# eglrp/PSBA

Measured on AMD Instinct MI355X. Metric: M-observations/sec through Jacobian+Schur build+solve (ms/LM-iter in ms_per_step), higher is better.
Workload: dtype f64; 1 GPU; venice-shaped; n_cams=52, n_pts=64053, n_obs=345364, lm=levmar, TR hand-off disabled, parallelism=points sharded x1

## Files before the change

### include/psba_hip.h

```cpp
#ifndef PSBA_HIP_H
#define PSBA_HIP_H

#ifdef __cplusplus
extern "C" {
#endif

typedef struct psba_ctx *psba_handle;

#define PSBA_OK 0
#define PSBA_NOT_SPD 1
#define PSBA_SINGULAR_V 2
#define PSBA_PCG_MAXIT 4
#define PSBA_E_INVALID (-1)
#define PSBA_E_HIP (-2)
#define PSBA_E_RCCL (-3)
#define PSBA_E_IO (-4)
#define PSBA_E_NOMEM (-5)
#define PSBA_E_STATE (-6)

#define PSBA_ITER_TURN_TO_LM 1
#define PSBA_ITER_TURN_TO_TR 2
#define PSBA_ITER_CONTINUE 3
#define PSBA_ITER_ERR 4
#define PSBA_ITER_DP_NO_CHANGE 5
// ... 117 lines not shown
int psba_set_step(psba_handle h, const double *dp);
int psba_cholmod_lambda(psba_handle h, int reassemble, double *lambda, double *info3);
int psba_get_cholmod_factor(psba_handle h, double *L);
int psba_get_free_obs_blocks(psba_handle h, double *W, double *Be);

typedef struct {
  int max_iter;
  int start_itno;
  int verbose;
  int log_cap;
  double init_lambda;
} psba_tr_options;

typedef struct {
  int flag;
  int iters;
  int tries;
  int chol_fail;
  double init_err, final_err, lambda, delta;
  int n_log;
  double seconds;
} psba_tr_result;

void psba_tr_default_options(psba_tr_options *o);
int psba_trust_region(psba_handle h, const psba_tr_options *opts, psba_tr_result *res, double *log);

typedef struct {
  int flag, iters, lm_calls, tr_calls;
  double init_err, final_err, seconds;
} psba_solve_result;
int psba_solve(psba_handle h, int max_iter, int verbose, psba_solve_result *res);

int psba_partition_points(int n3Dpts, const int *iidx, int n2Dprojs, int nranks, int *pt_begin);
int psba_comm_unique_id(void *id128);
int psba_comm_init(psba_handle h, int nranks, int rank, const void *id128);
int psba_comm_rank(psba_handle h, int *nranks, int *rank);
int psba_set_rank_layout(psba_handle h, int nranks, int rank);
int psba_reduce_buffer_size(psba_handle h, long long *n_doubles);
int psba_get_reduce_buffer(psba_handle h, double *out);
int psba_set_reduce_buffer(psba_handle h, const double *in);

typedef struct {
  int nCams, n3Dpts, n2Dprojs;
  double *Kparas, *impts, *initrot, *camsEx, *pts3D;
  int *iidx, *jidx;
} psba_problem;
int psba_read_problem(const char *cams_file, const char *pts_file, const double *fixedK,
                      psba_problem *out);
void psba_free_problem(psba_problem *p);
typedef struct {
  psba_problem base;
  double *kc, *cov;
} psba_problem_ex;
int psba_read_problem_ex(const char *cams_file, const char *pts_file, const double *fixedK, psba_problem_ex *out);
void psba_free_problem_ex(psba_problem_ex *p);
int psba_write_problem(const char *cams_file, const char *pts_file, int nCams, int n3Dpts, int n2Dprojs,
                       const double *Kparas, const double *initrot, const double *camsEx, const double *pts3D,
                       const double *impts, const int *iidx, const int *jidx, int with_K);
int psba_convert_bal(const char *bal_file, const char *cams_out, const char *pts_out, double *max_abs_k);
int psba_convert_bal_kd(const char *bal_file, const char *cams_out, const char *pts_out);

#define PSBA_K_LINEARIZE 0
#define PSBA_K_SCHUR 1
#define PSBA_K_CHOLESKY 2
#define PSBA_K_BACKSUB 3
#define PSBA_K_RESIDUAL 4
#define PSBA_K_ALLREDUCE 5
#define PSBA_K_SCHUR_REDUCE 6
#define PSBA_K_COUNT 7
int psba_profile_enable(psba_handle h, int on);
int psba_profile_reset(psba_handle h);
int psba_profile_get(psba_handle h, int kernel, double *total_ms, int *launches);
int psba_algorithmic_bytes(psba_handle h, int kernel, double *bytes);

#define PSBA_SOLVER_DENSE 0
#define PSBA_SOLVER_PCG 1
int psba_set_solver(psba_handle h, int solver, double tol, int max_iter);
int psba_pcg_info(psba_handle h, int *iters, double *relres, long long *blocks, long long *dense_blocks);
int psba_get_sparse_S(psba_handle h, int *jk, double *val, double *ea);
int psba_set_sparse_S(psba_handle h, const double *val, const double *ea);
int psba_sparse_pattern(int nCams, int n3Dpts, int n2Dprojs, const int *iidx, const int *jidx, unsigned char *flags);
int psba_set_sparse_pattern(psba_handle h, const unsigned char *flags, long long n);

int psba_chol_dist_shape(psba_handle h, int *n32, int *NB, int *sharded);
int psba_chol_shape(psba_handle h, int *out8);
int psba_chol_dist_exchange_plan(int n32, int NB, int nranks, int JE, long long *out4, int cap);
int psba_chol_dist_begin(psba_handle h);
int psba_chol_dist_superpanel(psba_handle h, int J);
int psba_chol_dist_block(psba_handle h, int B, int set, double *buf, long long *n_doubles);
int psba_chol_dist_finish(psba_handle h);

typedef struct psba_schur_plan *psba_schur_plan_t;
psba_schur_plan_t psba_schur_plan_create(int nCams, int n3Dpts, int n2Dprojs, const int *iidx,
                                         const int *jidx);
int psba_schur_plan_info(psba_schur_plan_t p, long long info[8]);
int psba_schur_plan_copy(psba_schur_plan_t p, unsigned long long *items, long long *wg,
                         int *blockpos, int *glo);
void psba_schur_plan_destroy(psba_schur_plan_t p);

typedef struct psba_owner_plan *psba_owner_plan_t;
psba_owner_plan_t psba_owner_plan_create(int nCams, int n3Dpts, int n2Dprojs, const int *iidx, const int *jidx,
                                         const unsigned char *pattern);
int psba_owner_plan_info(psba_owner_plan_t p, long long info[4]);
int psba_owner_plan_copy(psba_owner_plan_t p, long long *waves, int *units, int *prod, int *blocks, int *diag_slot);
void psba_owner_plan_destroy(psba_owner_plan_t p);

typedef struct psba_blockprod_plan *psba_blockprod_plan_t;
psba_blockprod_plan_t psba_blockprod_plan_create(int nCams, int n3Dpts, int n2Dprojs, const int *iidx, const int *jidx,
                                                 int seg_len);
int psba_blockprod_plan_info(psba_blockprod_plan_t p, long long info[4]);
int psba_blockprod_plan_copy(psba_blockprod_plan_t p, int *blocks, int *segs, int *prods);
void psba_blockprod_plan_destroy(psba_blockprod_plan_t p);

#ifdef PSBA_BUILD_EXPERIMENTS
typedef struct psba_ring_plan *psba_ring_plan_t;
psba_ring_plan_t psba_ring_plan_create(int nCams, int n3Dpts, int n2Dprojs, const int *iidx,
                                       const int *jidx);
int psba_ring_plan_info(psba_ring_plan_t p, long long info[16]);
int psba_ring_plan_copy(psba_ring_plan_t p, long long *wg, int *steps, unsigned *entries, int *ops,
                        int *jobs, int *lane_blk, int *blk_lane0, int *rb);
void psba_ring_plan_destroy(psba_ring_plan_t p);
#endif

#ifdef __cplusplus
}
#endif
#endif
```

### psba_amd/capi.py

```python
import ctypes as C
import os

import numpy as np

_HERE = os.path.dirname(os.path.abspath(__file__))
lib_path = os.environ.get("PSBA_LIB") or os.path.join(_HERE, "libpsba_hip.so")

if not os.path.exists(lib_path):
    raise ImportError(
        f"{lib_path} is missing: build the HIP extension first (python -m psba_amd.build, or "
        "__graft_entry__.build()). psba_amd has no CPU fallback.")
lib = C.CDLL(lib_path)

PSBA_OK, PSBA_NOT_SPD, PSBA_SINGULAR_V = 0, 1, 2
PARAMS_CUR, PARAMS_NEW = 0, 1
LOSS_NONE, LOSS_HUBER, LOSS_CAUCHY, LOSS_SOFT_L1 = 0, 1, 2, 3
CAMERA_FIXED_K, CAMERA_FREE_K, CAMERA_FREE_KD = 0, 1, 2
INTRINSICS_BAL = (1, 0, 0, 0, 0, 1, 1, 0, 0, 0)
ITER_TURN_TO_LM, ITER_TURN_TO_TR, ITER_CONTINUE, ITER_ERR = 1, 2, 3, 4
ITER_DP_NO_CHANGE, ITER_ERR_SMALL_ENOUGH, ITER_PASS = 5, 6, 7
K_LINEARIZE, K_SCHUR, K_CHOLESKY, K_BACKSUB, K_RESIDUAL, K_ALLREDUCE, K_SCHUR_REDUCE = range(7)
KERNEL_NAMES = ["linearize", "schur", "cholesky", "backsub", "residual", "allreduce", "schur_reduce"]

_h = C.c_void_p
# ... 41 lines not shown


class CProblemEx(C.Structure):
    _fields_ = [("base", CProblem), ("kc", _dp), ("cov", _dp)]


SIGNATURES = [
    ("psba_create", C.c_int, [C.c_int, C.POINTER(_h)]),
    ("psba_destroy", C.c_int, [_h]),
    ("psba_last_error", C.c_char_p, [_h]),
    ("psba_version", C.c_char_p, []),
    ("psba_upload_problem", C.c_int, [_h, C.c_int, C.c_int, C.c_int, _dp, _dp, _dp, _dp, _dp, _ip, _ip]),
    ("psba_set_params", C.c_int, [_h, _dp, _dp]),
    ("psba_reset_params", C.c_int, [_h]),
    ("psba_get_params", C.c_int, [_h, C.c_int, _dp, _dp]),
    ("psba_get_dims", C.c_int, [_h, _ip, _ip, _ip]),
    ("psba_schur_path", C.c_int, [_h, C.POINTER(C.c_int)]),
    ("psba_residual", C.c_int, [_h, C.c_int, _dp]),
    ("psba_linearize", C.c_int, [_h, C.c_double, C.c_double]),
    ("psba_max_diag", C.c_int, [_h, _dp]),
    ("psba_begin", C.c_int, [_h, C.c_double, C.c_double, _dp, _dp]),
    ("psba_schur_assemble", C.c_int, [_h, C.c_double]),
    ("psba_schur_reduce", C.c_int, [_h]),
    ("psba_schur_solve", C.c_int, [_h]),
    ("psba_backsub", C.c_int, [_h, C.c_double, C.POINTER(TryScalars)]),
    ("psba_backsub_async", C.c_int, [_h, C.c_double]),
    ("psba_linearize_ahead", C.c_int, [_h]),
    ("psba_backsub_wait", C.c_int, [_h, C.POINTER(TryScalars)]),
    ("psba_accept", C.c_int, [_h]),
    ("psba_compute_exQT", C.c_int, [_h, C.c_int, _dp]),
    ("psba_compute_jacobiQT", C.c_int, [_h, _dp, _dp]),
    ("psba_compute_U", C.c_int, [_h, C.c_double, _dp]),
    ("psba_compute_V", C.c_int, [_h, C.c_double, _dp]),
    ("psba_maxElmOfUV", C.c_int, [_h, _dp]),
    ("psba_update_UV", C.c_int, [_h, C.c_double, _dp, _dp]),
    ("psba_restore_UVdiag", C.c_int, [_h]),
    ("psba_compute_Vinv", C.c_int, [_h, _dp]),
    ("psba_compute_Wblks", C.c_int, [_h, C.c_double, _dp]),
    ("psba_compute_Yblks", C.c_int, [_h, _dp]),
    ("psba_compute_S", C.c_int, [_h, _dp]),
    ("psba_compute_g", C.c_int, [_h, C.c_double, _dp]),
    ("psba_compute_ea", C.c_int, [_h, _dp]),
    ("psba_SPDinv_matVec", C.c_int, [_h, _dp]),
    ("psba_compute_eb", C.c_int, [_h, _dp]),
    ("psba_compute_dpb", C.c_int, [_h, _dp]),
    ("psba_compute_newp", C.c_int, [_h, _dp]),
    ("psba_update_p", C.c_int, [_h, _dp]),
    ("psba_lm_default_options", None, [C.POINTER(LmOptions)]),
    ("psba_levmar", C.c_int, [_h, C.POINTER(LmOptions), C.POINTER(LmResult), _dp]),
    ("psba_partition_points", C.c_int, [C.c_int, _ip, C.c_int, C.c_int, _ip]),
    ("psba_comm_unique_id", C.c_int, [C.c_void_p]),
    ("psba_comm_init", C.c_int, [_h, C.c_int, C.c_int, C.c_void_p]),
    ("psba_comm_rank", C.c_int, [_h, _ip, _ip]),
    ("psba_set_rank_layout", C.c_int, [_h, C.c_int, C.c_int]),
    ("psba_reduce_buffer_size", C.c_int, [_h, C.POINTER(C.c_longlong)]),
    ("psba_get_reduce_buffer", C.c_int, [_h, _dp]),
    ("psba_set_reduce_buffer", C.c_int, [_h, _dp]),
    ("psba_read_problem", C.c_int, [C.c_char_p, C.c_char_p, _dp, C.POINTER(CProblem)]),
    ("psba_free_problem", None, [C.POINTER(CProblem)]),
    ("psba_profile_enable", C.c_int, [_h, C.c_int]),
    ("psba_profile_reset", C.c_int, [_h]),
    ("psba_profile_get", C.c_int, [_h, C.c_int, _dp, _ip]),
    ("psba_algorithmic_bytes", C.c_int, [_h, C.c_int, _dp]),
    ("psba_compute_Jmultiply", C.c_int, [_h, _dp, _dp]),
    ("psba_jmul_dots", C.c_int, [_h, _dp, _dp, _dp]),
    ("psba_get_gradient", C.c_int, [_h, _dp]),
    ("psba_get_dp", C.c_int, [_h, _dp]),
    ("psba_set_step", C.c_int, [_h, _dp]),
    ("psba_cholmod_lambda", C.c_int, [_h, C.c_int, _dp, _dp]),
    ("psba_get_cholmod_factor", C.c_int, [_h, _dp]),
    ("psba_get_free_obs_blocks", C.c_int, [_h, _dp, _dp]),
    ("psba_tr_default_options", None, [C.POINTER(TrOptions)]),
    ("psba_trust_region", C.c_int, [_h, C.POINTER(TrOptions), C.POINTER(TrResult), _dp]),
    ("psba_solve", C.c_int, [_h, C.c_int, C.c_int, C.POINTER(SolveResult)]),
    ("psba_write_problem", C.c_int, [C.c_char_p, C.c_char_p, C.c_int, C.c_int, C.c_int, _dp, _dp, _dp, _dp, _dp, _ip, _ip, C.c_int]),
    ("psba_convert_bal", C.c_int, [C.c_char_p, C.c_char_p, C.c_char_p, _dp]),
    ("psba_allreduce_scalars", C.c_int, [_h, _dp, C.c_int]),
    ("psba_set_solver", C.c_int, [_h, C.c_int, C.c_double, C.c_int]),
    ("psba_pcg_info", C.c_int, [_h, _ip, _dp, C.POINTER(C.c_longlong), C.POINTER(C.c_longlong)]),
    ("psba_get_sparse_S", C.c_int, [_h, _ip, _dp, _dp]),
    ("psba_set_sparse_S", C.c_int, [_h, _dp, _dp]),
    ("psba_sparse_pattern", C.c_int, [C.c_int, C.c_int, C.c_int, _ip, _ip, C.POINTER(C.c_ubyte)]),
    ("psba_set_sparse_pattern", C.c_int, [_h, C.POINTER(C.c_ubyte), C.c_longlong]),
    ("psba_set_camera_model", C.c_int, [_h, C.c_int]),
    ("psba_camera_block", C.c_int, [_h, _ip]),
    ("psba_set_distortion", C.c_int, [_h, _dp]),
    ("psba_set_obs_covariance", C.c_int, [_h, _dp]),
    ("psba_lens_model", C.c_int, [_h, _ip, _ip]),
    ("psba_set_robust_loss", C.c_int, [_h, C.c_int, C.c_double]),
    ("psba_robust_loss", C.c_int, [_h, _ip, _dp]),
    ("psba_obs_sq_residuals", C.c_int, [_h, C.c_int, _dp]),
    ("psba_set_fixed", C.c_int, [_h, C.POINTER(C.c_ubyte), C.POINTER(C.c_ubyte)]),
    ("psba_fixed_counts", C.c_int, [_h, _ip, _ip]),
    ("psba_read_problem_ex", C.c_int, [C.c_char_p, C.c_char_p, _dp, C.POINTER(CProblemEx)]),
    ("psba_free_problem_ex", None, [C.POINTER(CProblemEx)]),
    ("psba_convert_bal_kd", C.c_int, [C.c_char_p, C.c_char_p, C.c_char_p]),
    ("psba_chol_dist_exchange_plan", C.c_int, [C.c_int, C.c_int, C.c_int, C.c_int, C.POINTER(C.c_longlong), C.c_int]),
    ("psba_chol_dist_shape", C.c_int, [_h, _ip, _ip, _ip]),
    ("psba_chol_shape", C.c_int, [_h, _ip]),
    ("psba_chol_dist_begin", C.c_int, [_h]),
    ("psba_chol_dist_superpanel", C.c_int, [_h, C.c_int]),
    ("psba_chol_dist_block", C.c_int, [_h, C.c_int, C.c_int, _dp, C.POINTER(C.c_longlong)]),
    ("psba_chol_dist_finish", C.c_int, [_h]),
    ("psba_schur_plan_create", C.c_void_p, [C.c_int, C.c_int, C.c_int, _ip, _ip]),
    ("psba_schur_plan_info", C.c_int, [C.c_void_p, C.POINTER(C.c_longlong)]),
    ("psba_schur_plan_copy", C.c_int, [C.c_void_p, C.POINTER(C.c_ulonglong), C.POINTER(C.c_longlong), _ip, _ip]),
    ("psba_schur_plan_destroy", None, [C.c_void_p]),
    ("psba_owner_plan_create", C.c_void_p, [C.c_int, C.c_int, C.c_int, _ip, _ip, C.POINTER(C.c_ubyte)]),
    ("psba_owner_plan_info", C.c_int, [C.c_void_p, C.POINTER(C.c_longlong)]),
    ("psba_owner_plan_copy", C.c_int, [C.c_void_p, C.POINTER(C.c_longlong), _ip, _ip, _ip, _ip]),
    ("psba_owner_plan_destroy", None, [C.c_void_p]),
    ("psba_set_intrinsics_mask", C.c_int, [_h, C.POINTER(C.c_ubyte)]),
    ("psba_intrinsics_mask", C.c_int, [_h, C.POINTER(C.c_ubyte)]),
    ("psba_set_intrinsics_groups", C.c_int, [_h, C.POINTER(C.c_int)]),
    ("psba_intrinsics_groups", C.c_int, [_h, C.POINTER(C.c_int), C.POINTER(C.c_int)]),
    ("psba_blockprod_plan_create", C.c_void_p, [C.c_int, C.c_int, C.c_int, _ip, _ip, C.c_int]),
    ("psba_blockprod_plan_info", C.c_int, [C.c_void_p, C.POINTER(C.c_longlong)]),
    ("psba_blockprod_plan_copy", C.c_int, [C.c_void_p, _ip, _ip, _ip]),
    ("psba_blockprod_plan_destroy", None, [C.c_void_p]),
]
EXPERIMENT_SIGNATURES = [
    ("psba_ring_plan_create", C.c_void_p, [C.c_int, C.c_int, C.c_int, _ip, _ip]),
    ("psba_ring_plan_info", C.c_int, [C.c_void_p, C.POINTER(C.c_longlong)]),
    ("psba_ring_plan_copy", C.c_int, [C.c_void_p, C.POINTER(C.c_longlong), _ip, C.POINTER(C.c_uint), _ip, _ip, _ip, _ip, _ip]),
    ("psba_ring_plan_destroy", None, [C.c_void_p]),
]
HAS_EXPERIMENTS = hasattr(lib, "psba_ring_plan_create")
for _name, _res, _args in SIGNATURES + (EXPERIMENT_SIGNATURES if HAS_EXPERIMENTS else []):
    _f = getattr(lib, _name)
    _f.restype = _res
    _f.argtypes = _args


class PsbaError(RuntimeError):
    def __init__(self, code, msg):
        super().__init__(f"psba error {code}: {msg}")
        self.code = code


def _d(a):
    return None if a is None else a.ctypes.data_as(_dp)


def _i(a):
    return None if a is None else a.ctypes.data_as(_ip)


def _c(a, dt=np.float64):
    return np.ascontiguousarray(a, dtype=dt)


class Problem(dict):
    """K[nC,5] initrot[nC,4] cams[nC,6] pts[nP,3] impts[nO,2] iidx[nO] jidx[nO] nC nP nO.
    Optional: kc[nC,5], cov[nO,2,2] (read_problem_ex); fixed_cams[nC], fixed_pts[nP] (masks for Psba.set_fixed)."""


def sparse_pattern(prob):
    nC = int(prob["nC"])
    flags = np.zeros(nC * (nC + 1) // 2, dtype=np.uint8)
    ii = np.ascontiguousarray(prob["iidx"], dtype=np.int32)
    jj = np.ascontiguousarray(prob["jidx"], dtype=np.int32)
    rc = lib.psba_sparse_pattern(nC, int(prob["nP"]), int(prob["nO"]), _i(ii), _i(jj),
                                 flags.ctypes.data_as(C.POINTER(C.c_ubyte)))
    if rc != 0:
        raise PsbaError(rc, "psba_sparse_pattern failed")
    return flags


def _problem_from(cp):
    nC, nP, nO = cp.nCams, cp.n3Dpts, cp.n2Dprojs
    arr = lambda p, n, shape: np.ctypeslib.as_array(p, shape=(n,)).copy().reshape(shape)
    return Problem(K=arr(cp.Kparas, 5 * nC, (nC, 5)), initrot=arr(cp.initrot, 4 * nC, (nC, 4)),
                  cams=arr(cp.camsEx, 6 * nC, (nC, 6)), pts=arr(cp.pts3D, 3 * nP, (nP, 3)),
                  impts=arr(cp.impts, 2 * nO, (nO, 2)), iidx=arr(cp.iidx, nO, (nO,)).astype(np.int32),
                  jidx=arr(cp.jidx, nO, (nO,)).astype(np.int32), nC=nC, nP=nP, nO=nO)


def read_problem(cams_file, pts_file, fixedK=None):
    cp = CProblem()
    k = None if fixedK is None else _c(fixedK)
    rc = lib.psba_read_problem(os.fsencode(cams_file), os.fsencode(pts_file), _d(k), C.byref(cp))
    if rc != 0:
        raise PsbaError(rc, f"psba_read_problem({cams_file}, {pts_file}) failed")
    out = _problem_from(cp)
    lib.psba_free_problem(C.byref(cp))
    return out


def read_problem_ex(cams_file, pts_file, fixedK=None):
    cp = CProblemEx()
    k = None if fixedK is None else _c(fixedK)
    rc = lib.psba_read_problem_ex(os.fsencode(cams_file), os.fsencode(pts_file), _d(k), C.byref(cp))
    if rc != 0:
        raise PsbaError(rc, f"psba_read_problem_ex({cams_file}, {pts_file}) failed")
    out = _problem_from(cp.base)
    nC, nO = out["nC"], out["nO"]
    out["kc"] = np.ctypeslib.as_array(cp.kc, shape=(5 * nC,)).copy().reshape(nC, 5) if cp.kc else None
    out["cov"] = np.ctypeslib.as_array(cp.cov, shape=(4 * nO,)).copy().reshape(nO, 2, 2) if cp.cov else None
    lib.psba_free_problem_ex(C.byref(cp))
    return out


def write_problem(cams_file, pts_file, prob, cams=None, pts=None, with_K=True):
    c = _c(prob["cams"] if cams is None else cams)
    p = _c(prob["pts"] if pts is None else pts)
    K, rot, im = _c(prob["K"]), _c(prob["initrot"]), _c(prob["impts"])
    ii, jj = _c(prob["iidx"], np.int32), _c(prob["jidx"], np.int32)
    rc = lib.psba_write_problem(cams_file.encode(), pts_file.encode(), int(prob["nC"]), int(prob["nP"]),
                                int(prob["nO"]), _d(K), _d(rot), _d(c), _d(p), _d(im), _i(ii), _i(jj), int(with_K))
    if rc != 0:
        raise PsbaError(rc, f"psba_write_problem({cams_file}, {pts_file}) failed")


def convert_bal(bal_file, cams_out, pts_out):
    k = C.c_double()
    rc = lib.psba_convert_bal(bal_file.encode(), cams_out.encode(), pts_out.encode(), C.byref(k))
    if rc != 0:
        raise PsbaError(rc, f"psba_convert_bal({bal_file}) failed")
    return k.value


def convert_bal_kd(bal_file, cams_out, pts_out):
    rc = lib.psba_convert_bal_kd(bal_file.encode(), cams_out.encode(), pts_out.encode())
    if rc != 0:
        raise PsbaError(rc, f"psba_convert_bal_kd({bal_file}) failed")


def partition_points(n_pts, iidx, nranks):
    iidx = _c(iidx, np.int32)
    out = np.zeros(nranks + 1, dtype=np.int32)
    rc = lib.psba_partition_points(int(n_pts), _i(iidx), int(iidx.size), int(nranks), _i(out))
    if rc != 0:
        raise PsbaError(rc, "psba_partition_points failed")
    return out


def schur_plan(n_cams, n_pts, iidx, jidx):
    iidx = _c(iidx, np.int32)
    jidx = _c(jidx, np.int32)
    p = lib.psba_schur_plan_create(int(n_cams), int(n_pts), int(iidx.size), _i(iidx), _i(jidx))
    if not p:
        raise PsbaError(-1, "psba_schur_plan_create failed")
    try:
        info = (C.c_longlong * 8)()
        lib.psba_schur_plan_info(p, info)
        groups, nwg, nslots, products, slab, nblocks, run_tasks, pair_items = (int(x) for x in info)
        items = np.zeros(nslots, dtype=np.uint64)
        wg = np.zeros((nwg, 8), dtype=np.int64)
        blockpos = np.zeros(nblocks, dtype=np.int32)
        glo = np.zeros(groups + 1, dtype=np.int32)
        lib.psba_schur_plan_copy(p, items.ctypes.data_as(C.POINTER(C.c_ulonglong)),
                                 wg.ctypes.data_as(C.POINTER(C.c_longlong)), _i(blockpos), _i(glo))
    finally:
        lib.psba_schur_plan_destroy(p)
    return dict(groups=groups, items=items, wg=wg, blockpos=blockpos, glo=glo, products=products,
                slab_doubles=slab, run_tasks=run_tasks, pair_items=pair_items)


def owner_plan(n_cams, n_pts, iidx, jidx, pattern=None):
    iidx = _c(iidx, np.int32)
    jidx = _c(jidx, np.int32)
    pat = None if pattern is None else np.ascontiguousarray(pattern, dtype=np.uint8)
    pp = None if pat is None else pat.ctypes.data_as(C.POINTER(C.c_ubyte))
    p = lib.psba_owner_plan_create(int(n_cams), int(n_pts), int(iidx.size), _i(iidx), _i(jidx), pp)
    if not p:
        raise PsbaError(-1, "psba_owner_plan_create failed")
    try:
        info = (C.c_longlong * 4)()
        lib.psba_owner_plan_info(p, info)
        nw, rows, products, nblk = (int(x) for x in info)
        waves = np.zeros((nw, 2), dtype=np.int64)
        units = np.zeros((64 * nw, 4), dtype=np.int32)
        prod = np.zeros((64 * rows, 2), dtype=np.int32)
        blocks = np.zeros((nblk, 2), dtype=np.int32)
        diag = np.zeros(int(n_cams), dtype=np.int32)
        lib.psba_owner_plan_copy(p, waves.ctypes.data_as(C.POINTER(C.c_longlong)), _i(units), _i(prod), _i(blocks), _i(diag))
    finally:
        lib.psba_owner_plan_destroy(p)
    return dict(waves=waves, units=units, prod=prod.reshape(rows, 64, 2), blocks=blocks, diag_slot=diag, products=products)


def blockprod_plan(n_cams, n_pts, iidx, jidx, seg_len):
    iidx = _c(iidx, np.int32)
    jidx = _c(jidx, np.int32)
    p = lib.psba_blockprod_plan_create(int(n_cams), int(n_pts), int(iidx.size), _i(iidx), _i(jidx), int(seg_len))
    if not p:
        raise PsbaError(-1, "psba_blockprod_plan_create failed")
    try:
        info = (C.c_longlong * 4)()
        lib.psba_blockprod_plan_info(p, info)
        nb, ns, npr, tiles = (int(x) for x in info)
        blocks = np.zeros((nb, 2), dtype=np.int32)
        segs = np.zeros((ns, 3), dtype=np.int32)
        prods = np.zeros((npr, 2), dtype=np.int32)
        lib.psba_blockprod_plan_copy(p, _i(blocks), _i(segs), _i(prods))
    finally:
        lib.psba_blockprod_plan_destroy(p)
    return dict(blocks=blocks, segs=segs, prods=prods, tiles=tiles)


def chol_dist_exchange_plan(n32, NB, nranks, JE):
    out = np.zeros((64, 4), dtype=np.int64)
    n = lib.psba_chol_dist_exchange_plan(int(n32), int(NB), int(nranks), int(JE), out.ctypes.data_as(C.POINTER(C.c_longlong)), 64)
    if n < 0:
        raise PsbaError(n, "psba_chol_dist_exchange_plan failed")
    return [tuple(int(v) for v in row) for row in out[:n]]


def ring_plan(n_cams, n_pts, iidx, jidx):
    if not HAS_EXPERIMENTS:
# ... 146 lines not shown
        return c.value, p.value

    def obs_sq_residuals(self, which=PARAMS_CUR):
        return self._out(lib.psba_obs_sq_residuals, self.nO, which)[1]

    def camera_block(self):
        n = C.c_int()
        self._ck(lib.psba_camera_block(self._h, C.byref(n)))
        return n.value

    def upload_problem(self, prob):
        self.nC, self.nP, self.nO = int(prob["nC"]), int(prob["nP"]), int(prob["nO"])
        self.cnp = self.camera_block()
        self.nA, self.nB = self.cnp * self.nC, 3 * self.nP
        self.nT = self.nA + self.nB
        a = [_c(prob[k]).reshape(-1) for k in ("K", "impts", "initrot", "cams", "pts")]
        ii, jj = _c(prob["iidx"], np.int32), _c(prob["jidx"], np.int32)
        self._ck(lib.psba_upload_problem(self._h, self.nC, self.nP, self.nO, _d(a[0]), _d(a[1]),
                                         _d(a[2]), _d(a[3]), _d(a[4]), _i(ii), _i(jj)))

    def set_params(self, cams, pts):
        c, p = _c(cams).reshape(-1), _c(pts).reshape(-1)
        self._ck(lib.psba_set_params(self._h, _d(c), _d(p)))

    def reset_params(self):
        self._ck(lib.psba_reset_params(self._h))

    def get_params(self, which=PARAMS_CUR):
        c, p = np.empty(self.nA), np.empty(self.nB)
        self._ck(lib.psba_get_params(self._h, which, _d(c), _d(p)))
        return c.reshape(self.nC, self.cnp), p.reshape(self.nP, 3)

    def schur_path(self):
        v = C.c_int()
        self._ck(lib.psba_schur_path(self._h, C.byref(v)))
        return v.value

    def residual(self, which=PARAMS_CUR):
        v = C.c_double()
        self._ck(lib.psba_residual(self._h, which, C.byref(v)))
        return v.value

    def linearize(self, coeff=1.0, coeff_g=1.0):
        self._ck(lib.psba_linearize(self._h, coeff, coeff_g))

    def begin(self, coeff=1.0, coeff_g=1.0):
        c, m = C.c_double(), C.c_double()
        self._ck(lib.psba_begin(self._h, coeff, coeff_g, C.byref(c), C.byref(m)))
        return c.value, m.value

    def max_diag(self):
        v = C.c_double()
        self._ck(lib.psba_max_diag(self._h, C.byref(v)))
        return v.value

    def schur_assemble(self, mu):
        self._ck(lib.psba_schur_assemble(self._h, mu))

    def schur_reduce(self):
        self._ck(lib.psba_schur_reduce(self._h))

    def schur_solve(self):
        return self._ck(lib.psba_schur_solve(self._h))

    def backsub(self, mu):
        s = TryScalars()
        self._ck(lib.psba_backsub(self._h, mu, C.byref(s)))
        return s

    def backsub_async(self, mu):
        self._ck(lib.psba_backsub_async(self._h, mu))

    def linearize_ahead(self):
        self._ck(lib.psba_linearize_ahead(self._h))

    def backsub_wait(self):
        s = TryScalars()
        self._ck(lib.psba_backsub_wait(self._h, C.byref(s)))
        return s

    def accept(self):
        self._ck(lib.psba_accept(self._h))

    def _out(self, fn, n, *pre):
        out = np.empty(n)
        rc = self._ck(fn(self._h, *pre, _d(out)))
        return rc, out

    def compute_exQT(self, which=PARAMS_CUR):
        return self._out(lib.psba_compute_exQT, 2 * self.nO, which)[1]

    def compute_jacobiQT(self):
        JA, JB = np.empty(12 * self.nO), np.empty(6 * self.nO)
        self._ck(lib.psba_compute_jacobiQT(self._h, _d(JA), _d(JB)))
        return JA, JB

    def compute_U(self, coeff=1.0):
        return self._out(lib.psba_compute_U, 36 * self.nC, coeff)[1]

    def compute_V(self, coeff=1.0):
        return self._out(lib.psba_compute_V, 9 * self.nP, coeff)[1]

    def maxElmOfUV(self):
        v = C.c_double()
        self._ck(lib.psba_maxElmOfUV(self._h, C.byref(v)))
        return v.value

    def update_UV(self, mu):
        U, V = np.empty(36 * self.nC), np.empty(9 * self.nP)
        self._ck(lib.psba_update_UV(self._h, mu, _d(U), _d(V)))
        return U, V

    def restore_UVdiag(self):
        self._ck(lib.psba_restore_UVdiag(self._h))

    def compute_Vinv(self):
        return self._out(lib.psba_compute_Vinv, 9 * self.nP)

    def compute_Wblks(self, coeff=1.0):
        return self._out(lib.psba_compute_Wblks, 18 * self.nO, coeff)[1]

    def compute_Yblks(self):
        return self._out(lib.psba_compute_Yblks, 18 * self.nO)[1]

    def compute_S(self):
        return self._out(lib.psba_compute_S, self.nA * self.nA)[1].reshape(self.nA, self.nA)

    def compute_g(self, coeff=1.0):
        return self._out(lib.psba_compute_g, self.nT, coeff)[1]

    def compute_ea(self):
        return self._out(lib.psba_compute_ea, self.nA)[1]

    def SPDinv_matVec(self):
        return self._out(lib.psba_SPDinv_matVec, self.nA)

    def compute_eb(self):
        return self._out(lib.psba_compute_eb, self.nB)[1]

    def compute_dpb(self):
        return self._out(lib.psba_compute_dpb, self.nT)[1]

    def compute_newp(self):
        return self._out(lib.psba_compute_newp, self.nT)[1]

    def update_p(self):
        return self._out(lib.psba_update_p, self.nT)[1]

    def levmar(self, max_iter=50, tr_handoff=False, verbose=False, log_cap=512, start_itno=0, init_mu=0.0,
               stop_cost=0.0):
        opts = LmOptions(max_iter, int(tr_handoff), int(verbose), log_cap, start_itno, init_mu, stop_cost)
        res = LmResult()
        log = np.zeros((max(log_cap, 1), 5))
        self._ck(lib.psba_levmar(self._h, C.byref(opts), C.byref(res), _d(log)))
        return res, log[: res.n_log].copy()

    def set_solver(self, solver, tol=0.0, max_iter=0):
        self._ck(lib.psba_set_solver(self._h, int(solver), float(tol), int(max_iter)))

    def pcg_info(self):
        it, rr, nb, nd = C.c_int(), C.c_double(), C.c_longlong(), C.c_longlong()
        self._ck(lib.psba_pcg_info(self._h, C.byref(it), C.byref(rr), C.byref(nb), C.byref(nd)))
        return it.value, rr.value, nb.value, nd.value

    def get_sparse_S(self):
        nb = self.pcg_info()[2]
# ... 137 lines not shown
```

### psba_amd/csrc/kernels_backsub.hip

```cpp
#include <cstdlib>

#include "camera_model.h"
#include "psba_internal.h"

namespace psba {

struct BackArgs {
  const double *W, *PV, *camconst, *cams, *pts, *impts, *ga;
  const int *iidx, *jidx, *ptr;
  const int4 *tile_desc;
  double *dp;
  double *newcams, *newpts;
  double *scal;
  double *dbg_eb;
  const int *status;
  double mu;
  double coeff;
  int nC, nA, nTiles;
  int cam_terms;
  int mode;
  const double *kc, *wl;
};

template <bool DUMP, bool RECOMP, int LM>
// ... 249 lines not shown
    lens_load_w<LM>(p.wl, a, wl);
    const double2 m = reinterpret_cast<const double2 *>(p.impts)[a];
    lens_residual<LM>(cc, cam, sNP, kc, wl, m.x, m.y, e0, e1);
    s_cost += lens_cost<LM>(rl, e0, e1);
  }
  __syncthreads();
  {
    double v = s_cost;
#pragma unroll
    for (int off = 32; off > 0; off >>= 1) v += __shfl_down(v, off, 64);
    if ((tid & 63) == 0) sRed[tid >> 6][3] = v;
  }
  __syncthreads();
  if (tid == 0) {
    double c = 0.0;
    for (int w2 = 0; w2 < TILE_OBS / 64; w2++) c += sRed[w2][3];
    double *dst = p.scal + SC_PART + 4 * (blockIdx.x % SC_NPART);
    atomicAdd(&dst[0], s_dp);
    atomicAdd(&dst[1], s_den);
    atomicAdd(&dst[2], c);
    atomicAdd(&dst[3], s_np);
  }
}

__global__ __launch_bounds__(128) void k_publish_scal(const double *scal, double *host) {
  if (threadIdx.x < NSCAL) host[threadIdx.x] = scal[threadIdx.x];
}

int launch_publish_scal(psba_ctx *h, hipStream_t s) {
  hipLaunchKernelGGL(k_publish_scal, dim3(1), dim3(128), 0, s, h->scal, h->h_scal_dev);
  PSBA_HIP(h, hipGetLastError());
  return PSBA_OK;
}

__global__ __launch_bounds__(256) void k_struct_only_begin(const double *PV, double mu, int nA, int nP, double *dp, double *scal,
                                                           int *status, int try_id) {
  const int gtid = blockIdx.x * blockDim.x + threadIdx.x, gsize = gridDim.x * blockDim.x;
  if (blockIdx.x == 0 && threadIdx.x < 4 * SC_NPART) scal[SC_PART + threadIdx.x] = 0.0;
  if (blockIdx.x == 0 && threadIdx.x == 64) status[3] = try_id;
  for (int t = gtid; t < nA; t += gsize) dp[t] = 0.0;
  for (int i = gtid; i < nP; i += gsize) {
    double v[6], vi[6];
#pragma unroll
    for (int k = 0; k < 6; k++) v[k] = PV[9 * (size_t)i + k];
    v[0] += mu;
    v[3] += mu;
    v[5] += mu;
    if (sym3_inverse(v, vi)) status[0] = try_id;
  }
}

int launch_struct_only_try(psba_ctx *h, double mu) {
  h->try_id++;
  h->diag_done = false;
  h->packed_pending = false;
  int grid = (h->d.nP + 255) / 256;
  if (grid > 1024) grid = 1024;
  hipLaunchKernelGGL(k_struct_only_begin, dim3(grid), dim3(256), 0, h->stream, h->PV, mu, h->d.nA, h->d.nP, h->dp, h->scal,
                     h->status, h->try_id);
  PSBA_HIP(h, hipGetLastError());
  return PSBA_OK;
}

template <int LM>
static void enqueue_backsub(psba_ctx *h, const BackArgs &a, const RobustLoss &rl, const FixedMask &fm, int grid, bool dump, bool read_w) {
  if (dump && read_w)
    hipLaunchKernelGGL((k_backsub<true, false, LM>), dim3(grid), dim3(TILE_OBS), 0, h->stream, a, rl, fm);
  else if (dump)
    hipLaunchKernelGGL((k_backsub<true, true, LM>), dim3(grid), dim3(TILE_OBS), 0, h->stream, a, rl, fm);
  else if (read_w)
    hipLaunchKernelGGL((k_backsub<false, false, LM>), dim3(grid), dim3(TILE_OBS), 0, h->stream, a, rl, fm);
  else
    hipLaunchKernelGGL((k_backsub<false, true, LM>), dim3(grid), dim3(TILE_OBS), 0, h->stream, a, rl, fm);
  if (h->nLong) {
    if (dump)
      hipLaunchKernelGGL((k_backsub_long<true, LM>), dim3(h->nLong), dim3(TILE_OBS), 0, h->stream, a, h->long_pts, rl, fm);
    else
      hipLaunchKernelGGL((k_backsub_long<false, LM>), dim3(h->nLong), dim3(TILE_OBS), 0, h->stream, a, h->long_pts, rl, fm);
  }
}

int launch_backsub(psba_ctx *h, double mu, bool dump) {
  if (h->cnp != 6) return dump ? mirror_refused(h) : launch_backsub_free(h, mu);
  const Dims &d = h->d;
  BackArgs a;
  a.W = h->W;
  a.PV = h->PV;
  a.camconst = h->camconst;
  a.cams = h->cams[h->cur];
  a.pts = h->pts[h->cur];
  a.impts = h->impts;
  a.ga = h->ga;
  a.iidx = h->iidx;
  a.jidx = h->jidx;
  a.ptr = h->ptr;
  a.tile_desc = h->tile_desc;
  a.dp = h->dp;
  a.newcams = h->cams[1 - h->cur];
  a.newpts = h->pts[1 - h->cur];
  a.scal = h->scal;
  a.dbg_eb = h->dbg_eb;
  a.status = h->status;
  a.mu = mu;
  a.coeff = h->coeff_w;
  a.nC = d.nC;
  a.nA = d.nA;
  a.nTiles = d.nTiles;
  a.cam_terms = h->rank == 0 ? 1 : 0;
  a.kc = h->lens_kc;
  a.wl = h->lens_w;
  const RobustLoss rl = make_robust_loss(h->loss_kind, h->loss_c);
  {
    const char *m = getenv("PSBA_BACK_MODE");
    a.mode = m ? atoi(m) : 0;
  }
  if (dump) PSBA_HIP(h, hipMemsetAsync(h->scal + SC_PART, 0, 4 * SC_NPART * sizeof(double), h->stream));
  int grid = d.nTiles < 768 ? d.nTiles : 768;
  if (const char *e = getenv("PSBA_BACK_GRID")) grid = atoi(e) > 0 && atoi(e) < grid ? atoi(e) : grid;
  {
    ProfScope ps(h, PSBA_K_BACKSUB);
    const bool read_w = getenv("PSBA_BACK_READ_W") != nullptr;
    const FixedMask fm = {h->fix_cams, h->fix_pts};
    lens_dispatch_fixed(h->lens, h->has_fixed, [&](auto m) { enqueue_backsub<decltype(m)::value>(h, a, rl, fm, grid, dump, read_w); });
  }
  PSBA_HIP(h, hipGetLastError());
  return PSBA_OK;
}

}
```

### psba_amd/csrc/kernels_linearize.hip

```cpp
#include <cstdlib>

#include "camera_model.h"
#include "psba_internal.h"

namespace psba {

struct LinArgs {
  const double *camconst, *cams, *pts, *impts;
  const int *iidx, *jidx, *ptr;
  const int4 *tile_desc;
  double *W, *PV, *campart;
  double *camacc;
  double *dbg_ex, *dbg_JA, *dbg_JB;
  double coeff, coeff_g;
  int nC, nTiles;
  int mode;
  const double *pub_src;
  double *pub_dst;
  double pub_stamp;
  const double *kc, *wl;
};

template <bool DUMP, bool GACC, int LM>
__global__ __launch_bounds__(TILE_OBS) void k_linearize(LinArgs p, RobustLoss rl, FixedMask fm) {
// ... 476 lines not shown
  __shared__ double sRed[4];
  double sum = 0.0;
  for (int a = blockIdx.x * blockDim.x + threadIdx.x; a < nO; a += gridDim.x * blockDim.x) {
    const int i = iidx[a], j = jidx[a];
    double cc[9], cam[6], M[3], e0, e1, kc[5], wl[3];
#pragma unroll
    for (int k = 0; k < 9; k++) cc[k] = camconst[9 * j + k];
#pragma unroll
    for (int k = 0; k < 6; k++) cam[k] = cams[6 * j + k];
#pragma unroll
    for (int k = 0; k < 3; k++) M[k] = pts[3 * i + k];
    lens_load_kc<LM>(kcs, j, kc);
    lens_load_w<LM>(wls, a, wl);
    const double2 m = reinterpret_cast<const double2 *>(impts)[a];
    lens_residual<LM>(cc, cam, M, kc, wl, m.x, m.y, e0, e1);
    const double f = lens_cost<LM>(rl, e0, e1, s_out ? s_out + a : nullptr);
    if (ex_out) {
      ex_out[2 * a] = e0;
      ex_out[2 * a + 1] = e1;
    }
    sum += f;
  }
#pragma unroll
  for (int off = 32; off > 0; off >>= 1) sum += __shfl_down(sum, off, 64);
  if ((threadIdx.x & 63) == 0) sRed[threadIdx.x >> 6] = sum;
  __syncthreads();
  if (threadIdx.x == 0) atomicAdd(cost, sRed[0] + sRed[1] + sRed[2] + sRed[3]);
}

__global__ __launch_bounds__(256) void k_max_diag(const double *U, const double *PV, int nC,
                                                  int nP, double *out) {
  __shared__ double sRed[4];
  double m = 0.0;
  const int gtid = blockIdx.x * blockDim.x + threadIdx.x, gsize = gridDim.x * blockDim.x;
  for (int t = gtid; t < 6 * nC; t += gsize) m = fmax(m, U[36 * (t / 6) + 7 * (t % 6)]);
  for (int i = gtid; i < nP; i += gsize) {
    const double *v = PV + 9 * (size_t)i;
    m = fmax(m, fmax(v[0], fmax(v[3], v[5])));
  }
#pragma unroll
  for (int off = 32; off > 0; off >>= 1) m = fmax(m, __shfl_down(m, off, 64));
  if ((threadIdx.x & 63) == 0) sRed[threadIdx.x >> 6] = m;
  __syncthreads();
  if (threadIdx.x == 0) {
    m = fmax(fmax(sRed[0], sRed[1]), fmax(sRed[2], sRed[3]));
    atomicMax(reinterpret_cast<unsigned long long *>(out),
              (unsigned long long)__double_as_longlong(m));
  }
}

__global__ __launch_bounds__(256) void k_max_diag_fixed(const double *U, const double *PV, int nC, int nP, double *out,
                                                        FixedMask fm) {
  __shared__ double sRed[4];
  double m = 0.0;
  const int gtid = blockIdx.x * blockDim.x + threadIdx.x, gsize = gridDim.x * blockDim.x;
  for (int t = gtid; t < 6 * nC; t += gsize)
    if (!(fm.cams && fm.cams[t / 6])) m = fmax(m, U[36 * (t / 6) + 7 * (t % 6)]);
  for (int i = gtid; i < nP; i += gsize) {
    if (fm.pts && fm.pts[i]) continue;
    const double *v = PV + 9 * (size_t)i;
    m = fmax(m, fmax(v[0], fmax(v[3], v[5])));
  }
#pragma unroll
  for (int off = 32; off > 0; off >>= 1) m = fmax(m, __shfl_down(m, off, 64));
  if ((threadIdx.x & 63) == 0) sRed[threadIdx.x >> 6] = m;
  __syncthreads();
  if (threadIdx.x == 0) {
    m = fmax(fmax(sRed[0], sRed[1]), fmax(sRed[2], sRed[3]));
    atomicMax(reinterpret_cast<unsigned long long *>(out), (unsigned long long)__double_as_longlong(m));
  }
}

template <int LM>
static int set_lin_attrs(psba_ctx *h) {
  const auto attr = hipFuncAttributeMaxDynamicSharedMemorySize;
  PSBA_HIP(h, hipFuncSetAttribute((const void *)k_linearize<true, false, LM>, attr, 100 * 1024));
  PSBA_HIP(h, hipFuncSetAttribute((const void *)k_linearize<false, false, LM>, attr, 100 * 1024));
  PSBA_HIP(h, hipFuncSetAttribute((const void *)k_linearize2<true, false, LM>, attr, 100 * 1024));
  PSBA_HIP(h, hipFuncSetAttribute((const void *)k_linearize2<false, false, LM>, attr, 100 * 1024));
  return PSBA_OK;
}

template <int LM>
static void enqueue_linearize(psba_ctx *h, const LinArgs &a, const RobustLoss &rl, const FixedMask &fm, bool dump, bool v1, size_t lds, double *Uo, double *gao) {
  const Dims &d = h->d;
  if (h->cam_global) {
    const int grid = d.nTiles < 2048 ? d.nTiles : 2048;
    if (v1 && dump)
      hipLaunchKernelGGL((k_linearize<true, true, LM>), dim3(grid), dim3(TILE_OBS), 0, h->stream, a, rl, fm);
    else if (v1)
      hipLaunchKernelGGL((k_linearize<false, true, LM>), dim3(grid), dim3(TILE_OBS), 0, h->stream, a, rl, fm);
    else if (dump)
      hipLaunchKernelGGL((k_linearize2<true, true, LM>), dim3(grid), dim3(TILE_OBS), 0, h->stream, a, rl, fm);
    else
      hipLaunchKernelGGL((k_linearize2<false, true, LM>), dim3(grid), dim3(TILE_OBS), 0, h->stream, a, rl, fm);
    if (h->nLong) {
      if (dump)
        hipLaunchKernelGGL((k_linearize_long<true, true, LM>), dim3(h->nLong), dim3(TILE_OBS), 0, h->stream, a, h->long_pts, (double *)nullptr, rl, fm);
      else
        hipLaunchKernelGGL((k_linearize_long<false, true, LM>), dim3(h->nLong), dim3(TILE_OBS), 0, h->stream, a, h->long_pts, (double *)nullptr, rl, fm);
    }
    hipLaunchKernelGGL(k_cam_sums<LM>, dim3((h->nCamUnits + 3) / 4), dim3(256), 0, h->stream, a, h->cam_obs,
                       h->cam_units, h->nCamUnits, rl, fm);
    hipLaunchKernelGGL(k_cam_finalize, dim3((42 * d.nC + 255) / 256), dim3(256), 0, h->stream, h->camacc, d.nC,
                       h->coeff, h->coeff_g, Uo, gao);
  } else {
    if (v1 && dump)
      hipLaunchKernelGGL((k_linearize<true, false, LM>), dim3(h->nPart), dim3(TILE_OBS), lds, h->stream, a, rl, fm);
    else if (v1)
      hipLaunchKernelGGL((k_linearize<false, false, LM>), dim3(h->nPart), dim3(TILE_OBS), lds, h->stream, a, rl, fm);
    else if (dump)
      hipLaunchKernelGGL((k_linearize2<true, false, LM>), dim3(h->nPart), dim3(TILE_OBS), lds, h->stream, a, rl, fm);
    else
      hipLaunchKernelGGL((k_linearize2<false, false, LM>), dim3(h->nPart), dim3(TILE_OBS), lds, h->stream, a, rl, fm);
    int nslab = h->nPart;
    if (h->nLong) {
      double *slab = h->campart + (size_t)h->nPart * d.nC * CAM_ACC;
      if (dump)
        hipLaunchKernelGGL((k_linearize_long<true, false, LM>), dim3(h->nLong), dim3(TILE_OBS), 0, h->stream, a, h->long_pts, slab, rl, fm);
      else
        hipLaunchKernelGGL((k_linearize_long<false, false, LM>), dim3(h->nLong), dim3(TILE_OBS), 0, h->stream, a, h->long_pts, slab, rl, fm);
      nslab++;
    }
    hipLaunchKernelGGL(k_cam_reduce, dim3(d.nC), dim3(1024), 0, h->stream, h->campart, nslab, d.nC, h->coeff,
                       h->coeff_g, Uo, gao);
  }
}

int launch_linearize(psba_ctx *h, bool dump, bool ahead, bool publish) {
  if (h->cnp != 6) return dump ? mirror_refused(h) : launch_linearize_free(h, ahead, publish);
  const Dims &d = h->d;
  LinArgs a;
  a.camconst = h->camconst;
  const int set = ahead ? 1 - h->cur : h->cur;
  a.cams = h->cams[set];
  a.pts = h->pts[set];
  a.impts = h->impts;
  a.iidx = h->iidx;
  a.jidx = h->jidx;
  a.ptr = h->ptr;
  a.tile_desc = h->tile_desc;
  a.W = ahead ? h->W_alt : h->W;
  a.PV = ahead ? h->PV_alt : h->PV;
  a.campart = h->campart;
  a.camacc = h->camacc;
  a.dbg_ex = h->dbg_ex;
  a.dbg_JA = h->dbg_JA;
  a.dbg_JB = h->dbg_JB;
  a.coeff = h->coeff;
  h->coeff_w = h->coeff;
  a.coeff_g = h->coeff_g;
  a.nC = d.nC;
  a.nTiles = d.nTiles;
  a.pub_src = h->scal;
  a.pub_dst = publish ? h->h_scal_dev : nullptr;
  a.pub_stamp = h->pub_seq;
  a.kc = h->lens_kc;
  a.wl = h->lens_w;
  const RobustLoss rl = make_robust_loss(h->loss_kind, h->loss_c);
  const FixedMask fm = {h->fix_cams, h->fix_pts};
  {
    const char *m = getenv("PSBA_LIN_MODE");
    a.mode = m ? atoi(m) : 0;
  }
  const bool v1 = getenv("PSBA_LIN_V1") != nullptr;
  const size_t lds = h->cam_global ? 0 : sizeof(double) * CAM_ACC * (size_t)d.nC;
  if (!h->lin_attr_set && lds > 8 * 1024) {
    int rc = PSBA_OK;
    for (int lm = 0; lm < 2 * LENS_MODELS && rc == PSBA_OK; lm++)
      lens_dispatch_fixed(lm % LENS_MODELS, lm >= LENS_MODELS, [&](auto m) { rc = set_lin_attrs<decltype(m)::value>(h); });
    if (rc != PSBA_OK) return rc;
    h->lin_attr_set = true;
  }
  double *Uo = ahead ? h->U_alt : h->U, *gao = ahead ? h->ga_alt : h->ga;
  {
    ProfScope ps(h, PSBA_K_LINEARIZE);
    if (h->cam_global)
      PSBA_HIP(h, hipMemsetAsync(h->camacc, 0, sizeof(double) * CAM_ACC * (size_t)d.nC, h->stream));
    else if (h->nLong)
      PSBA_HIP(h, hipMemsetAsync(h->campart + (size_t)h->nPart * d.nC * CAM_ACC, 0, sizeof(double) * CAM_ACC * (size_t)d.nC,
                                 h->stream));
    lens_dispatch_fixed(h->lens, h->has_fixed, [&](auto m) { enqueue_linearize<decltype(m)::value>(h, a, rl, fm, dump, v1, lds, Uo, gao); });
    if (h->has_fixed)
      hipLaunchKernelGGL(k_fixed_diag, dim3((d.nC + d.nP + 255) / 256), dim3(256), 0, h->stream, fm, d.nC, d.nP, h->coeff,
                         h->rank == 0 ? h->coeff : 0.0, Uo, gao, a.PV);
  }
  PSBA_HIP(h, hipGetLastError());
  return PSBA_OK;
}

int launch_residual(psba_ctx *h, int which, double *ex_out_dev, double *s_out_dev) {
  if (h->cnp != 6) return ex_out_dev || s_out_dev ? mirror_refused(h) : launch_residual_free(h, which);
  const Dims &d = h->d;
  const int set = which == PSBA_PARAMS_NEW ? 1 - h->cur : h->cur;
  PSBA_HIP(h, hipMemsetAsync(h->scal + SC_COST, 0, sizeof(double), h->stream));
  int grid = (d.nO + 255) / 256;
  if (grid > 256) grid = 256;
  {
    ProfScope ps(h, PSBA_K_RESIDUAL);
    const RobustLoss rl = make_robust_loss(h->loss_kind, h->loss_c);
    lens_dispatch(h->lens | (s_out_dev ? LENS_ROBUST : 0), [&](auto m) {
      hipLaunchKernelGGL(k_residual<decltype(m)::value>, dim3(grid), dim3(256), 0, h->stream, h->camconst, h->cams[set],
                         h->pts[set], h->impts, h->iidx, h->jidx, d.nO, ex_out_dev, h->scal + SC_COST, h->lens_kc,
                         h->lens_w, rl, s_out_dev);
    });
  }
  PSBA_HIP(h, hipGetLastError());
  return PSBA_OK;
}

int launch_max_diag(psba_ctx *h) {
  if (h->cnp != 6) return launch_max_diag_free(h);
  PSBA_HIP(h, hipMemsetAsync(h->scal + SC_MAXDIAG, 0, sizeof(double), h->stream));
  int grid = (h->d.nP + 255) / 256;
  if (grid > 512) grid = 512;
  if (h->has_fixed)
    hipLaunchKernelGGL(k_max_diag_fixed, dim3(grid), dim3(256), 0, h->stream, h->U, h->PV, h->d.nC, h->d.nP,
                       h->scal + SC_MAXDIAG, FixedMask{h->fix_cams, h->fix_pts});
  else
    hipLaunchKernelGGL(k_max_diag, dim3(grid), dim3(256), 0, h->stream, h->U, h->PV, h->d.nC, h->d.nP,
                       h->scal + SC_MAXDIAG);
  PSBA_HIP(h, hipGetLastError());
  return PSBA_OK;
}

}
```

### psba_amd/csrc/kernels_schur.hip

```cpp
#include "camera_model.h"
#include <cstdlib>

#include "schur_common.h"
#include "schur_lds_args.h"

namespace psba {

struct SchurArgs {
  const double *W, *PV;
  const int *iidx, *jidx, *ptr, *tile_pt;
  double *S, *ea;
  int *status;
  double *dbg_Y, *dbg_Vinv;
  double mu;
  int nC, nA, nTiles;
  int ld;
  int try_id;
};

template <bool DUMP>
__global__ __launch_bounds__(TILE_OBS) void k_schur_atomic(SchurArgs p) {
  __shared__ double sW[TILE_OBS * 18];
  __shared__ double sVi[TILE_OBS][9];
  __shared__ int sJ[TILE_OBS];
// ... 99 lines not shown
    const int ja = p.jidx[a];
    const double *w = p.W + 18 * (size_t)a;
    double Y[18];
#pragma unroll
    for (int r = 0; r < 6; r++) {
      const double w0 = w[3 * r], w1 = w[3 * r + 1], w2 = w[3 * r + 2];
      Y[3 * r] = w0 * vi[0] + w1 * vi[1] + w2 * vi[2];
      Y[3 * r + 1] = w0 * vi[1] + w1 * vi[3] + w2 * vi[4];
      Y[3 * r + 2] = w0 * vi[2] + w1 * vi[4] + w2 * vi[5];
      atomicAdd(&p.ea[6 * ja + r], -(Y[3 * r] * g0 + Y[3 * r + 1] * g1 + Y[3 * r + 2] * g2));
    }
    if (DUMP) {
#pragma unroll
      for (int k = 0; k < 18; k++) p.dbg_Y[18 * (size_t)a + k] = Y[k];
    }
    for (int b = o0; b <= a; b++) {
      double *Sblk = p.S + (size_t)(6 * ja) * p.ld + 6 * p.jidx[b];
      const double *wb = p.W + 18 * (size_t)b;
#pragma unroll
      for (int c = 0; c < 6; c++) {
        const double w0 = wb[3 * c], w1 = wb[3 * c + 1], w2 = wb[3 * c + 2];
#pragma unroll
        for (int r = 0; r < 6; r++)
          atomicAdd(&Sblk[(size_t)r * p.ld + c], -(Y[3 * r] * w0 + Y[3 * r + 1] * w1 + Y[3 * r + 2] * w2));
      }
    }
  }
}



template <bool DUMP>
__device__ __forceinline__ void schur_a_side(const SchurLdsArgs &p, int a, int i, double (&v)[6], double g0, double g1,
                                             double g2, const double (&w)[18], double (&Y)[18], double (&e)[6],
                                             bool dump_y) {
  double vi[6];
  v[0] += p.mu;
  v[3] += p.mu;
  v[5] += p.mu;
  if (sym3_inverse(v, vi)) p.status[0] = p.try_id;
  if (DUMP) {
    double *o = p.dbg_Vinv + 9 * (size_t)i;
    o[0] = vi[0]; o[1] = vi[1]; o[2] = vi[2];
    o[3] = vi[1]; o[4] = vi[3]; o[5] = vi[4];
    o[6] = vi[2]; o[7] = vi[4]; o[8] = vi[5];
  }
#pragma unroll
  for (int k = 0; k < 6; k++) vi[k] = -vi[k];
#pragma unroll
  for (int r = 0; r < 6; r++) {
    const double w0 = w[3 * r], w1 = w[3 * r + 1], w2 = w[3 * r + 2];
    Y[3 * r] = w0 * vi[0] + w1 * vi[1] + w2 * vi[2];
    Y[3 * r + 1] = w0 * vi[1] + w1 * vi[3] + w2 * vi[4];
    Y[3 * r + 2] = w0 * vi[2] + w1 * vi[4] + w2 * vi[5];
    e[r] = Y[3 * r] * g0 + Y[3 * r + 1] * g1 + Y[3 * r + 2] * g2;
  }
  if (DUMP && dump_y) {
#pragma unroll
    for (int k = 0; k < 18; k++) p.dbg_Y[18 * (size_t)a + k] = -Y[k];
  }
}

__device__ __forceinline__ void schur_block_add(double *blk, const double (&Y)[18], const double (&wb)[18], bool self,
                                                const double (&e)[6]) {
#pragma unroll
  for (int r = 0; r < 6; r++) {
    double val[6];
#pragma unroll
    for (int c = 0; c < 6; c++) val[c] = Y[3 * r] * wb[3 * c];
#pragma unroll
    for (int c = 0; c < 6; c++) val[c] = fma(Y[3 * r + 1], wb[3 * c + 1], val[c]);
#pragma unroll
    for (int c = 0; c < 6; c++) val[c] = fma(Y[3 * r + 2], wb[3 * c + 2], val[c]);
#pragma unroll
    for (int c = 0; c < 6; c++) {
      if (r == 0 && c >= 1) val[c] = self ? e[c - 1] : val[c];
      if (r == 1 && c == 2) val[c] = self ? e[5] : val[c];
    }
#pragma unroll
    for (int c = 0; c < 6; c++) atomicAdd(&blk[6 * r + c], val[c]);
  }
}

template <bool DUMP>
__global__ __launch_bounds__(SCHUR_THREADS) void k_schur_lds(SchurLdsArgs p) {
  extern __shared__ double sPart[];
  const int tid = threadIdx.x;
  int w = blockIdx.x;
  if ((p.nWg & 7) == 0) w = (blockIdx.x & 7) * (p.nWg >> 3) + (blockIdx.x >> 3);
  const SchurWg wg = p.wg[w];
  for (int t = tid; t < BLK_STRIDE * wg.nblk; t += SCHUR_THREADS) sPart[t] = 0.0;
  __syncthreads();

#ifdef PSBA_BUILD_EXPERIMENTS
  {
    const long long s1 = wg.itemD;
    unsigned long long item_next = (wg.item0 + tid < s1) ? p.items[wg.item0 + tid] : SCHUR_NULL_ITEM;
    for (long long t = wg.item0 + tid; t < s1; t += SCHUR_THREADS) {
      const unsigned long long item = item_next;
      if (t + SCHUR_THREADS < s1) item_next = p.items[t + SCHUR_THREADS];
      if (item == SCHUR_NULL_ITEM) continue;
      const int a = wg.obs0 + (int)(item & ((1u << PAIR_OBS_BITS) - 1));
      const int i = wg.pt0 + (int)((item >> PAIR_OBS_BITS) & ((1u << PAIR_PT_BITS) - 1));
      const int boff = (int)((item >> (PAIR_OBS_BITS + PAIR_PT_BITS)) & ((1u << ITEM_BOFF_BITS) - 1));
      const int pos = (int)((item >> (PAIR_OBS_BITS + PAIR_PT_BITS + ITEM_BOFF_BITS)) & ((1u << ITEM_POS_BITS) - 1));
      const int pos2 = (int)((item >> (PAIR_OBS_BITS + PAIR_PT_BITS + ITEM_BOFF_BITS + ITEM_POS_BITS)) & ((1u << ITEM_POS_BITS) - 1));
      const double *pv = p.PV + 9 * (size_t)i;
      const double2 *wa = reinterpret_cast<const double2 *>(p.W + 18 * (size_t)a);
      const double2 *wb2 = reinterpret_cast<const double2 *>(p.W + 18 * (size_t)(a - boff));
      double v[6], w[18], wb[18];
#pragma unroll
      for (int k = 0; k < 6; k++) v[k] = pv[k];
      const double g0 = pv[6], g1 = pv[7], g2 = pv[8];
#pragma unroll
      for (int k = 0; k < 9; k++) {
        const double2 q = wa[k];
        w[2 * k] = q.x;
        w[2 * k + 1] = q.y;
      }
#pragma unroll
      for (int k = 0; k < 9; k++) {
        const double2 q = wb2[k];
        wb[2 * k] = q.x;
        wb[2 * k + 1] = q.y;
      }
      double Y[18], e[6];
      schur_a_side<DUMP>(p, a, i, v, g0, g1, g2, w, Y, e, boff == 1);
      schur_block_add(sPart + BLK_STRIDE * pos, Y, wb, false, e);
      asm volatile("" ::: "memory");
#pragma unroll
      for (int k = 0; k < 9; k++) {
        const double2 q = wb2[9 + k];
        wb[2 * k] = q.x;
        wb[2 * k + 1] = q.y;
      }
      schur_block_add(sPart + BLK_STRIDE * pos2, Y, wb, boff == 1, e);
    }
  }
#endif
  const long long s1 = wg.item1;
  unsigned long long item_next = (wg.itemD + tid < s1) ? p.items[wg.itemD + tid] : SCHUR_NULL_ITEM;
  for (long long t = wg.itemD + tid; t < s1; t += SCHUR_THREADS) {
    const unsigned long long item = item_next;
    if (t + SCHUR_THREADS < s1) item_next = p.items[t + SCHUR_THREADS];
    if (item == SCHUR_NULL_ITEM) continue;
    const int a = wg.obs0 + (int)(item & ((1u << ITEM_OBS_BITS) - 1));
    const int i = wg.pt0 + (int)((item >> ITEM_OBS_BITS) & ((1u << ITEM_PT_BITS) - 1));
    const int boff = (int)((item >> (ITEM_OBS_BITS + ITEM_PT_BITS)) & ((1u << ITEM_BOFF_BITS) - 1));
    const int pos = (int)(item >> (ITEM_OBS_BITS + ITEM_PT_BITS + ITEM_BOFF_BITS));
    const double *pv = p.PV + 9 * (size_t)i;
    const double2 *wa = reinterpret_cast<const double2 *>(p.W + 18 * (size_t)a);
    const double2 *wb2 = reinterpret_cast<const double2 *>(p.W + 18 * (size_t)(a - boff));
    double v[6], w[18], wb[18];
#pragma unroll
    for (int k = 0; k < 6; k++) v[k] = pv[k];
    const double g0 = pv[6], g1 = pv[7], g2 = pv[8];
#pragma unroll
    for (int k = 0; k < 9; k++) {
      const double2 q = wa[k];
      w[2 * k] = q.x;
      w[2 * k + 1] = q.y;
    }
#pragma unroll
    for (int k = 0; k < 9; k++) {
      const double2 q = wb2[k];
      wb[2 * k] = q.x;
      wb[2 * k + 1] = q.y;
    }
    const bool self = boff == 0;
    double Y[18], e[6];
    schur_a_side<DUMP>(p, a, i, v, g0, g1, g2, w, Y, e, self);
    schur_block_add(sPart + BLK_STRIDE * pos, Y, wb, self, e);
  }
  __syncthreads();
  double2 *slab = reinterpret_cast<double2 *>(p.slab + wg.slab_off);
  for (int t = tid; t < 18 * wg.nblk; t += SCHUR_THREADS) {
    const double *src = sPart + BLK_STRIDE * (t / 18) + 2 * (t % 18);
    slab[t] = make_double2(src[0], src[1]);
  }
  if (p.diag0 && tid < 21 * 36) {
    const int b = tid / 36, rc = tid % 36;
    if (p.diag_grp[b] == wg.group) {
      const double v = sPart[BLK_STRIDE * p.diag_pos[b] + rc];
      if (v != 0.0) atomicAdd(&p.diag0[tid], v);
    }
  }
}

template <bool DUMP>
__global__ __launch_bounds__(RUN_THREADS) void k_schur_lds_runs(SchurLdsArgs p) {
  extern __shared__ double sPart[];
  const int tid = threadIdx.x;
  int w = blockIdx.x;
  if ((p.nWg & 7) == 0) w = (blockIdx.x & 7) * (p.nWg >> 3) + (blockIdx.x >> 3);
  const SchurWg wg = p.wg[w];
  for (int t = tid; t < BLK_STRIDE * wg.nblk; t += RUN_THREADS) sPart[t] = 0.0;
  __syncthreads();
  double acc[36];
#pragma unroll
  for (int k = 0; k < 36; k++) acc[k] = 0.0;
  int cur = -1;
  unsigned long long item_next = (wg.item0 + tid < wg.item1) ? p.items[wg.item0 + tid] : SCHUR_NULL_ITEM;
  for (long long t = wg.item0 + tid; t < wg.item1; t += RUN_THREADS) {
    const unsigned long long item = item_next;
    if (t + RUN_THREADS < wg.item1) item_next = p.items[t + RUN_THREADS];
    if (item == SCHUR_NULL_ITEM) continue;
    const int a = wg.obs0 + (int)(item & ((1u << ITEM_OBS_BITS) - 1));
    const int i = wg.pt0 + (int)((item >> ITEM_OBS_BITS) & ((1u << ITEM_PT_BITS) - 1));
    const int boff = (int)((item >> (ITEM_OBS_BITS + ITEM_PT_BITS)) & ((1u << ITEM_BOFF_BITS) - 1));
    const int pos = (int)(item >> (ITEM_OBS_BITS + ITEM_PT_BITS + ITEM_BOFF_BITS));
    const double *pv = p.PV + 9 * (size_t)i;
    const double2 *wa = reinterpret_cast<const double2 *>(p.W + 18 * (size_t)a);
    const double2 *wb2 = reinterpret_cast<const double2 *>(p.W + 18 * (size_t)(a - boff));
    double v[6], vi[6], wv[18], wb[18];
#pragma unroll
    for (int k = 0; k < 6; k++) v[k] = pv[k];
    const double g0 = pv[6], g1 = pv[7], g2 = pv[8];
#pragma unroll
    for (int k = 0; k < 9; k++) {
      const double2 q = wa[k];
      wv[2 * k] = q.x;
      wv[2 * k + 1] = q.y;
    }
#pragma unroll
    for (int k = 0; k < 9; k++) {
      const double2 q = wb2[k];
      wb[2 * k] = q.x;
      wb[2 * k + 1] = q.y;
    }
    if (pos != cur) {
      if (cur >= 0) {
        double *blk = sPart + BLK_STRIDE * cur;
#pragma unroll
        for (int k = 0; k < 36; k++) atomicAdd(&blk[k], acc[k]);
      }
#pragma unroll
      for (int k = 0; k < 36; k++) acc[k] = 0.0;
      cur = pos;
    }
    v[0] += p.mu;
    v[3] += p.mu;
    v[5] += p.mu;
    if (sym3_inverse(v, vi)) p.status[0] = p.try_id;
    if (DUMP) {
      double *o = p.dbg_Vinv + 9 * (size_t)i;
      o[0] = vi[0]; o[1] = vi[1]; o[2] = vi[2];
      o[3] = vi[1]; o[4] = vi[3]; o[5] = vi[4];
      o[6] = vi[2]; o[7] = vi[4]; o[8] = vi[5];
    }
    const bool self = boff == 0;
#pragma unroll
    for (int k = 0; k < 6; k++) vi[k] = -vi[k];
    double Y[18], e[6];
#pragma unroll
    for (int r = 0; r < 6; r++) {
      const double w0 = wv[3 * r], w1 = wv[3 * r + 1], w2 = wv[3 * r + 2];
      Y[3 * r] = w0 * vi[0] + w1 * vi[1] + w2 * vi[2];
      Y[3 * r + 1] = w0 * vi[1] + w1 * vi[3] + w2 * vi[4];
      Y[3 * r + 2] = w0 * vi[2] + w1 * vi[4] + w2 * vi[5];
      e[r] = Y[3 * r] * g0 + Y[3 * r + 1] * g1 + Y[3 * r + 2] * g2;
    }
    if (DUMP && self) {
#pragma unroll
      for (int k = 0; k < 18; k++) p.dbg_Y[18 * (size_t)a + k] = -Y[k];
    }
#pragma unroll
    for (int r = 0; r < 6; r++)
#pragma unroll
      for (int c = 0; c < 6; c++) {
        double val = fma(Y[3 * r + 2], wb[3 * c + 2], fma(Y[3 * r + 1], wb[3 * c + 1], Y[3 * r] * wb[3 * c]));
        if (r == 0 && c >= 1) val = self ? e[c - 1] : val;
        if (r == 1 && c == 2) val = self ? e[5] : val;
        acc[6 * r + c] += val;
      }
  }
  if (cur >= 0) {
    double *blk = sPart + BLK_STRIDE * cur;
#pragma unroll
    for (int k = 0; k < 36; k++) atomicAdd(&blk[k], acc[k]);
  }
// ... 200 lines not shown
  for (int t = 0; t < wv.len; t++) {
    const int2 nxt = t + 1 < wv.len ? pr[(size_t)(t + 1) * 64] : make_int2(-1, -1);
    if (ab.x >= 0) {
      const int i = p.iidx[ab.x];
      const double *pv = p.PV + 9 * (size_t)i;
      const double2 *wa = reinterpret_cast<const double2 *>(p.W + 18 * (size_t)ab.x);
      const double2 *wb2 = reinterpret_cast<const double2 *>(p.W + 18 * (size_t)ab.y);
      double v[6], vi[6], wr[18], wb[18];
#pragma unroll
      for (int q = 0; q < 6; q++) v[q] = pv[q];
      const double g0 = pv[6], g1 = pv[7], g2 = pv[8];
#pragma unroll
      for (int q = 0; q < 9; q++) {
        const double2 x = wa[q], y = wb2[q];
        wr[2 * q] = x.x;
        wr[2 * q + 1] = x.y;
        wb[2 * q] = y.x;
        wb[2 * q + 1] = y.y;
      }
      v[0] += p.mu;
      v[3] += p.mu;
      v[5] += p.mu;
      if (sym3_inverse(v, vi)) p.status[0] = p.try_id;
      double Y[18];
#pragma unroll
      for (int r = 0; r < 6; r++) {
        const double w0 = wr[3 * r], w1 = wr[3 * r + 1], w2 = wr[3 * r + 2];
        Y[3 * r] = w0 * vi[0] + w1 * vi[1] + w2 * vi[2];
        Y[3 * r + 1] = w0 * vi[1] + w1 * vi[3] + w2 * vi[4];
        Y[3 * r + 2] = w0 * vi[2] + w1 * vi[4] + w2 * vi[5];
      }
      if (diag) {
#pragma unroll
        for (int r = 0; r < 6; r++) ea[r] -= Y[3 * r] * g0 + Y[3 * r + 1] * g1 + Y[3 * r + 2] * g2;
      }
#pragma unroll
      for (int r = 0; r < 6; r++)
#pragma unroll
        for (int c = 0; c < 6; c++)
          acc[6 * r + c] -= Y[3 * r] * wb[3 * c] + Y[3 * r + 1] * wb[3 * c + 1] + Y[3 * r + 2] * wb[3 * c + 2];
    }
    ab = nxt;
  }
  if (un.slot < 0) return;
  const int ldb = p.bsr ? 6 : p.ld;
  double *Sb = p.bsr ? p.S + 36 * (size_t)un.slot : p.S + (size_t)(6 * un.j) * p.ld + 6 * un.k;
  if (un.multi) {
#pragma unroll
    for (int r = 0; r < 6; r++)
#pragma unroll
      for (int c = 0; c < 6; c++) atomicAdd(&Sb[(size_t)r * ldb + c], acc[6 * r + c]);
  } else {
#pragma unroll
    for (int r = 0; r < 6; r++)
#pragma unroll
      for (int c = 0; c < 6; c++) Sb[(size_t)r * ldb + c] = acc[6 * r + c];
  }
  if (diag) {
#pragma unroll
    for (int r = 0; r < 6; r++) atomicAdd(&p.ea[6 * un.j + r], ea[r]);
  }
}

static int launch_schur_lds(psba_ctx *h, double mu, bool dump) {
  const Dims &d = h->d;
  SchurLdsArgs a;
  a.W = h->W;
  a.PV = h->PV;
  a.wg = h->wg;
  a.items = h->items;
  a.slab = h->slab;
  a.status = h->status;
  a.dbg_Y = h->dbg_Y;
  a.dbg_Vinv = h->dbg_Vinv;
  a.mu = mu;
  a.nWg = h->nWg;
  a.try_id = h->try_id;
  const bool fuse_diag = h->nranks == 1 && h->diag0 && !getenv("PSBA_CHOL_SEPARATE_DIAG") &&
                         !getenv("PSBA_SCHUR_NO_FLUSH_DIAG");
  a.diag0 = fuse_diag ? h->diag0 : nullptr;
  for (int b = 0; b < 21; b++) {
    a.diag_grp[b] = h->h_diaggrp[b];
    a.diag_pos[b] = h->h_diagpos[b];
  }
  SchurReduceArgs r;
  r.slab = h->slab;
  r.U = h->U;
  r.ga = h->ga;
  r.posblock = h->posblock;
  r.S = h->red;
  r.ea = h->red + (size_t)h->n32 * h->n32;
  r.scal = h->scal;
  r.status = h->status;
  r.mu_add = h->rank == 0 ? mu : 0.0;
  r.pad_one = h->rank == 0 ? 1.0 : 0.0;
  r.nA = d.nA;
  r.n32 = h->n32;
  r.nGroups = h->nGroups;
  r.try_id = h->try_id;
  r.diag0 = h->diag0;
  r.packed = (h->comm || (h->nranks > 1 && getenv("PSBA_SCHUR_PACKED"))) ? h->redp : nullptr;
  h->packed_pending = r.packed != nullptr;
  r.Lx = h->chol_L;
  r.linv = h->chol_ws;
  r.ring_copies = 0;
  r.ring_stride = 0;
  int worst = 0;
  long long npos = 0;
  for (int g = 0; g < h->nGroups; g++) {
    npos += h->gnblk[g];
    if (h->gnblk[g] > worst) worst = h->gnblk[g];
  }
  const size_t lds = sizeof(double) * BLK_STRIDE * (size_t)worst;
  int most = 1;
  for (int g = 0; g < h->nGroups; g++) most = h->gnwg[g] > most ? h->gnwg[g] : most;
  r.grp16 = h->gtab;
  r.chunks = most > 4 ? 4 : 8;
  if (const char *e = getenv("PSBA_REDUCE_CHUNKS")) r.chunks = atoi(e) == 2 || atoi(e) == 4 || atoi(e) == 8 ? atoi(e) : 1;
  r.nchunks = 36 * npos / 64;
  const int rgrid = (int)((r.nchunks + r.chunks - 1) / r.chunks);
  r.diag_wg = fuse_diag ? rgrid : -1;
  const bool pair = (h->prof & (1u << PSBA_K_SCHUR)) && !(h->prof & (1u << PSBA_K_SCHUR_REDUCE));
  {
    ProfScope pp(h, pair ? PSBA_K_SCHUR : -1);
    {
      ProfScope ps(h, pair ? -1 : PSBA_K_SCHUR);
      const char *m = getenv("PSBA_SCHUR_MODE");
      const int mode = m ? atoi(m) : 0;
      const dim3 G(h->nWg), B(SCHUR_THREADS);
      bool launched = false;
      if (h->schur_runs) {
        const dim3 Br(RUN_THREADS);
        if (dump)
          hipLaunchKernelGGL((k_schur_lds_runs<true>), G, Br, lds, h->stream, a);
        else
          hipLaunchKernelGGL((k_schur_lds_runs<false>), G, Br, lds, h->stream, a);
        launched = true;
      }
#ifdef PSBA_BUILD_EXPERIMENTS
      if (!launched && !dump && mode > 0 && !h->schur_pairs) launched = launch_schur_lds_mode(mode, G, B, lds, h->stream, a);
#endif
      (void)mode;
      if (launched) {
      } else if (dump)
        hipLaunchKernelGGL((k_schur_lds<true>), G, B, lds, h->stream, a);
      else
        hipLaunchKernelGGL((k_schur_lds<false>), G, B, lds, h->stream, a);
    }
    PSBA_HIP(h, hipGetLastError());
    {
      ProfScope ps(h, pair ? -1 : PSBA_K_SCHUR_REDUCE);
      hipLaunchKernelGGL(k_schur_reduce, dim3(rgrid + (r.diag_wg >= 0 ? 1 : 0)), dim3(256), 0, h->stream, r);
    }
  }
  h->diag_done = r.diag_wg >= 0;
  PSBA_HIP(h, hipGetLastError());
  return PSBA_OK;
}

static int launch_schur_sparse(psba_ctx *h, double mu) {
  PSBA_HIP(h, hipMemsetAsync(h->bs_val, 0, sizeof(double) * ((size_t)36 * h->bs_nblk + h->d.nA), h->stream));
  SchurOwnerArgs o;
  o.W = h->W;
  o.PV = h->PV;
  o.iidx = h->iidx;
  o.prod = h->own_prod;
  o.waves = h->own_waves;
  o.units = h->own_units;
  o.S = h->bs_val;
  o.ea = h->bs_ea;
  o.status = h->status;
  o.mu = mu;
  o.nWaves = h->own_nwaves;
  o.ld = 6;
  o.try_id = h->try_id;
  o.bsr = 1;
  const bool pair = (h->prof & (1u << PSBA_K_SCHUR)) && !(h->prof & (1u << PSBA_K_SCHUR_REDUCE));
  {
    ProfScope pp(h, pair ? PSBA_K_SCHUR : -1);
    {
      ProfScope ps(h, pair ? -1 : PSBA_K_SCHUR);
      hipLaunchKernelGGL(k_schur_owner, dim3((h->own_nwaves + 3) / 4), dim3(256), 0, h->stream, o);
    }
    {
      ProfScope ps(h, pair ? -1 : PSBA_K_SCHUR_REDUCE);
      const int rc = launch_bsr_finalize(h, mu);
      if (rc != PSBA_OK) return rc;
    }
  }
  PSBA_HIP(h, hipGetLastError());
  return PSBA_OK;
}

int launch_schur(psba_ctx *h, double mu, bool dump) {
  if (h->cnp != 6) return dump ? mirror_refused(h) : launch_schur_free(h, mu);
  h->try_id++;
  h->diag_done = false;
  h->packed_pending = false;
  if (h->solver == PSBA_SOLVER_PCG) {
    if (dump) return fail(h, PSBA_E_INVALID, "the sba_func.h mirror verbs need the dense S: PSBA_SOLVER_DENSE");
    return launch_schur_sparse(h, mu);
  }
#ifdef PSBA_BUILD_EXPERIMENTS
  if (h->ring_nWg > 0 && !getenv("PSBA_SCHUR_ATOMIC")) return launch_schur_ring(h, mu, dump);
#endif
  if (h->nGroups > 0 && !getenv("PSBA_SCHUR_ATOMIC")) {
    if (!h->lds_attr_set) {
      const int dyn = 163840 - 256;
      const auto attr = hipFuncAttributeMaxDynamicSharedMemorySize;
      PSBA_HIP(h, hipFuncSetAttribute((const void *)k_schur_lds<true>, attr, dyn));
      PSBA_HIP(h, hipFuncSetAttribute((const void *)k_schur_lds<false>, attr, dyn));
      PSBA_HIP(h, hipFuncSetAttribute((const void *)k_schur_lds_runs<true>, attr, dyn));
      PSBA_HIP(h, hipFuncSetAttribute((const void *)k_schur_lds_runs<false>, attr, dyn));
      h->lds_attr_set = true;
    }
    return launch_schur_lds(h, mu, dump);
  }
  const Dims &d = h->d;
  SchurArgs a;
  a.W = h->W;
  a.PV = h->PV;
  a.iidx = h->iidx;
  a.jidx = h->jidx;
  a.ptr = h->ptr;
  a.tile_pt = h->tile_pt;
  a.S = h->red;
  a.ea = h->red + (size_t)h->n32 * h->n32;
  a.ld = h->n32;
  a.status = h->status;
  a.dbg_Y = h->dbg_Y;
  a.dbg_Vinv = h->dbg_Vinv;
  a.mu = mu;
  a.nC = d.nC;
  a.nA = d.nA;
  a.nTiles = d.nTilesAll;
  a.try_id = h->try_id;
  PSBA_HIP(h, hipMemsetAsync(h->red, 0, sizeof(double) * (size_t)(h->n32 + 1) * h->n32, h->stream));
  const bool owner = h->own_nwaves > 0 && !dump && !getenv("PSBA_SCHUR_ATOMIC");
  int grid = d.nTilesAll < 2048 ? d.nTilesAll : 2048;
  const size_t lds = sizeof(double) * (size_t)d.nA;
  if (!owner && lds > 100 * 1024)
    return fail(h, PSBA_E_INVALID, "global-atomic S assembly: 6 nCams = %d needs %zu B of LDS for e_a (> 100 KiB)",
                d.nA, lds);
  if (!owner && !h->atomic_attr_set && lds > 8 * 1024) {
    const auto attr = hipFuncAttributeMaxDynamicSharedMemorySize;
    PSBA_HIP(h, hipFuncSetAttribute((const void *)k_schur_atomic<true>, attr, 100 * 1024));
    PSBA_HIP(h, hipFuncSetAttribute((const void *)k_schur_atomic<false>, attr, 100 * 1024));
    h->atomic_attr_set = true;
  }
  const bool pair = (h->prof & (1u << PSBA_K_SCHUR)) && !(h->prof & (1u << PSBA_K_SCHUR_REDUCE));
  const double mu_add = h->rank == 0 ? mu : 0.0;
  size_t n2 = (size_t)d.nA * d.nA;
  size_t fg = (n2 + 255) / 256;
  const int fgrid = fg > 4096 ? 4096 : (int)fg;
  {
    ProfScope pp(h, pair ? PSBA_K_SCHUR : -1);
    {
      ProfScope ps(h, pair ? -1 : PSBA_K_SCHUR);
      if (owner) {
        SchurOwnerArgs o;
        o.W = h->W;
        o.PV = h->PV;
        o.iidx = h->iidx;
        o.prod = h->own_prod;
        o.waves = h->own_waves;
        o.units = h->own_units;
        o.S = a.S;
        o.ea = a.ea;
        o.status = h->status;
        o.mu = mu;
        o.nWaves = h->own_nwaves;
        o.ld = h->n32;
        o.try_id = h->try_id;
        o.bsr = 0;
        hipLaunchKernelGGL(k_schur_owner, dim3((h->own_nwaves + 3) / 4), dim3(256), 0, h->stream, o);
      } else {
        if (dump)
          hipLaunchKernelGGL(k_schur_atomic<true>, dim3(grid), dim3(TILE_OBS), lds, h->stream, a);
        else
          hipLaunchKernelGGL(k_schur_atomic<false>, dim3(grid), dim3(TILE_OBS), lds, h->stream, a);
        if (h->nLong) {
// ... 19 lines not shown
```

### psba_amd/csrc/kernels_tr.hip

```cpp
#include <hip/hip_cooperative_groups.h>

#include "camera_model.h"
#include "psba_internal.h"

namespace psba {

struct JmulArgs {
  const double *camconst, *cams, *pts, *impts;
  const int *iidx, *jidx;
  const double *x1, *x2;
  double *out1;
  double *dots;
  int nO, nA;
  const double *kc, *wl;
};

template <int LM>
__global__ __launch_bounds__(256) void k_jmul(JmulArgs p, RobustLoss rl, FixedMask fm) {
  __shared__ double sRed[3][4];
  double d11 = 0.0, d12 = 0.0, d22 = 0.0;
  for (int a = blockIdx.x * blockDim.x + threadIdx.x; a < p.nO; a += gridDim.x * blockDim.x) {
    const int i = p.iidx[a], j = p.jidx[a];
    double cc[9], cam[6], M[3], e[2], A[12], B[6], kc[5], wl[3];
#pragma unroll
// ... 423 lines not shown
      d = fmax(fabs(d), delta);
      double ljj = sqrt(d);
      int over = 0;
      double theta = 0.0;
      for (int i = j + 1 + gtid; i < n; i += GT) {
        double cij = M[(size_t)i * ld + j];
        for (int k = 0; k < j; k++) cij -= M[(size_t)i * ld + k] * M[(size_t)j * ld + k];
        C[i] = cij;
        const double l = cij / ljj;
        M[(size_t)i * ld + j] = l;
        M[(size_t)j * ld + i] = 0.0;
        if (l > beta) over = 1;
        theta = fmax(theta, fabs(cij));
      }
      if (over) atomicOr(ov1 + j, 1);
      theta = wave_max(theta);
      if ((tid & 63) == 0 && theta > 0.0) atomicMax(th + j, bits(theta));
      grid.sync();
      if (*(volatile int *)(ov1 + j)) {
        ljj = peek(th + j) / beta;
        for (int i = j + 1 + gtid; i < n; i += GT) M[(size_t)i * ld + j] = C[i] / ljj;
      }
      if (gtid == 0) M[(size_t)j * ld + j] = ljj;
      grid.sync();
    }
  }
  grid.sync();
  double e = 0.0;
  for (int i = gtid; i < n; i += GT) {
    double s = 0.0;
    for (int k = 0; k <= i; k++) s += M[(size_t)i * ld + k] * M[(size_t)i * ld + k];
    e += s - dg[i];
  }
#pragma unroll
  for (int off = 32; off > 0; off >>= 1) e += __shfl_xor(e, off, 64);
  if ((tid & 63) == 0) sRed[tid >> 6] = e;
  __syncthreads();
  if (tid == 0) {
    double s = 0.0;
    for (int w = 0; w < CMG_THREADS / 64; w++) s += sRed[w];
    part[blockIdx.x] = s;
  }
  grid.sync();
  if (gtid == 0) {
    double s = 0.0;
    for (unsigned b = 0; b < gridDim.x; b++) s += ((volatile double *)part)[b];
    out[0] = fabs(s) / n;
    out[1] = delta;
    out[2] = beta;
    out[3] = (double)single;
  }
}

int launch_jmul(psba_ctx *h, const double *x1_dev, const double *x2_dev, double *out1_dev, double *dots_dev) {
  JmulArgs a;
  a.camconst = h->camconst;
  a.cams = h->cams[h->cur];
  a.pts = h->pts[h->cur];
  a.impts = h->impts;
  a.iidx = h->iidx;
  a.jidx = h->jidx;
  a.x1 = x1_dev;
  a.x2 = x2_dev ? x2_dev : x1_dev;
  a.out1 = out1_dev;
  a.dots = dots_dev;
  a.nO = h->d.nO;
  a.nA = h->d.nA;
  a.kc = h->lens_kc;
  a.wl = h->lens_w;
  const RobustLoss rl = make_robust_loss(h->loss_kind, h->loss_c);
  PSBA_HIP(h, hipMemsetAsync(dots_dev, 0, 3 * sizeof(double), h->stream));
  int grid = (h->d.nO + 255) / 256;
  if (grid > 1024) grid = 1024;
  const FixedMask fm = {h->fix_cams, h->fix_pts};
  lens_dispatch_fixed(h->lens, h->has_fixed, [&](auto m) {
    hipLaunchKernelGGL(k_jmul<decltype(m)::value>, dim3(grid), dim3(256), 0, h->stream, a, rl, fm);
  });
  PSBA_HIP(h, hipGetLastError());
  return PSBA_OK;
}

int launch_pack_g(psba_ctx *h, double *g_dev) {
  const size_t n = (size_t)h->d.nT;
  hipLaunchKernelGGL(k_pack_g, dim3((unsigned)((n + 255) / 256)), dim3(256), 0, h->stream, h->ga, h->PV, h->d.nA, h->d.nP,
                     g_dev);
  PSBA_HIP(h, hipGetLastError());
  return PSBA_OK;
}

int launch_newp(psba_ctx *h, double *dp_dev) {
  const size_t n = (size_t)h->d.nT;
  if (h->has_fixed)
    hipLaunchKernelGGL(k_newp_fixed, dim3((unsigned)((n + 255) / 256)), dim3(256), 0, h->stream, h->cams[h->cur], h->pts[h->cur],
                       dp_dev, h->d.nA, h->d.nB, h->cams[1 - h->cur], h->pts[1 - h->cur], FixedMask{h->fix_cams, h->fix_pts});
  else
    hipLaunchKernelGGL(k_newp, dim3((unsigned)((n + 255) / 256)), dim3(256), 0, h->stream, h->cams[h->cur], h->pts[h->cur],
                     dp_dev, h->d.nA, h->d.nB, h->cams[1 - h->cur], h->pts[1 - h->cur]);
  PSBA_HIP(h, hipGetLastError());
  return PSBA_OK;
}

int launch_cholmod(psba_ctx *h, double *out4_dev) {
  const int n = h->d.nA, ld = h->n32;
  double *M = h->chol_L, *aux = h->chol_L + (size_t)(h->n32 + 1) * ld;
  if ((size_t)5 * n > (size_t)(h->n32 + 15) * ld) return fail(h, PSBA_E_INVALID, "cholmod scratch too small");
  PSBA_HIP(h, hipMemcpyAsync(M, h->red, sizeof(double) * (size_t)n * ld, hipMemcpyDeviceToDevice, h->stream));
  const char *force = getenv("PSBA_CHOLMOD_GRID");
  const bool use_grid = force ? atoi(force) != 0 : n >= 300;
  if (use_grid) {
    int nwg = (n + CMG_THREADS - 1) / CMG_THREADS;
    if (nwg > 256) nwg = 256;
    const int nJ = n / 3;
    double *gs = aux + 5 * (size_t)n;
    const size_t gs_doubles = 10 + (size_t)(nJ + 2 + n + 1) / 2 + 1 + (n + 2) + nwg;
    if ((size_t)5 * n + gs_doubles > (size_t)(h->n32 + 15) * ld) return fail(h, PSBA_E_INVALID, "cholmod scratch too small");
    PSBA_HIP(h, hipMemsetAsync(gs, 0, sizeof(double) * gs_doubles, h->stream));
    int ld_ = ld, n_ = n;
    void *args[] = {&M, &ld_, &n_, &aux, &out4_dev, &gs};
    PSBA_HIP(h, hipLaunchCooperativeKernel((const void *)k_cholmod_grid, dim3(nwg), dim3(CMG_THREADS), args, 0, h->stream));
    return PSBA_OK;
  }
  hipLaunchKernelGGL(k_cholmod, dim3(1), dim3(CM_THREADS), 0, h->stream, M, ld, n, aux, out4_dev);
  PSBA_HIP(h, hipGetLastError());
  return PSBA_OK;
}

}
```

### psba_amd/csrc/psba_api.cpp

```cpp
#include <algorithm>
#include <cmath>
#include <cstdarg>
#include <cstdio>
#include <cstdlib>
#include <cstring>
#include <string>
#include <new>
#include <vector>

#include "camera_model.h"
#include "psba_internal.h"

using namespace psba;

static thread_local std::string g_create_err;

namespace psba {

int fail(psba_ctx *h, int code, const char *fmt, ...) {
  char buf[1024];
  va_list ap;
  va_start(ap, fmt);
  vsnprintf(buf, sizeof buf, fmt, ap);
  va_end(ap);
  if (h)
    h->err = buf;
  else
    g_create_err = buf;
  return code;
}

int mirror_refused(psba_ctx *h) {
  return fail(h, PSBA_E_STATE, "the sba_func.h mirror is six-parameter only (not PSBA_CAMERA_FREE_K / PSBA_CAMERA_FREE_KD)");
}

ProfScope::ProfScope(psba_ctx *hh, int kind) : h(hh) {
  if (kind < 0 || !(h->prof & (1u << kind))) return;
  if (h->spans_used == h->spans.size()) {
    psba_ctx::Span s;
    s.kind = kind;
    if (hipEventCreateWithFlags(&s.a, hipEventDisableSystemFence) != hipSuccess ||
        hipEventCreateWithFlags(&s.b, hipEventDisableSystemFence) != hipSuccess)
      return;
    h->spans.push_back(s);
  }
  idx = (int)h->spans_used++;
  h->spans[idx].kind = kind;
  (void)hipEventRecord(h->spans[idx].a, h->stream);
}
ProfScope::~ProfScope() {
  if (idx >= 0) (void)hipEventRecord(h->spans[idx].b, h->stream);
}

}

#define CHECK_H_NOJOIN(h)                 \
  do {                                    \
    if (!(h)) return PSBA_E_INVALID;      \
    (void)hipSetDevice((h)->device);      \
  } while (0)
#define CHECK_H(h)                                                         \
  do {                                                                     \
    CHECK_H_NOJOIN(h);                                                     \
    if ((h)->scal_side) {                                                  \
      (void)hipStreamWaitEvent((h)->stream, (h)->scal_event, 0);           \
      (h)->scal_side = false;                                              \
    }                                                                      \
  } while (0)
#define NEED(h, cond, what)                                             \
  do {                                                                  \
    if (!(cond)) return fail((h), PSBA_E_STATE, "%s: %s", __func__, what); \
  } while (0)
#define SIX_ONLY "six-parameter camera blocks only (PSBA_CAMERA_FREE_K / PSBA_CAMERA_FREE_KD: the fused verbs and psba_levmar)"
#define NEED_SIX(h) NEED(h, (h)->cnp == 6, SIX_ONLY)
#define RCCL(h, call)                                                                   \
  do {                                                                                  \
    ncclResult_t r__ = (call);                                                          \
    if (r__ != ncclSuccess)                                                             \
      return fail((h), PSBA_E_RCCL, "%s failed: %s", #call, ncclGetErrorString(r__));   \
  } while (0)
#define TRY(expr)                 \
  do {                            \
    int rc__ = (expr);            \
    if (rc__ < 0) return rc__;    \
  } while (0)

namespace psba {
int alloc_bytes(psba_ctx *h, void **p, size_t bytes, bool pinned) {
  *p = nullptr;
  if (pinned) {
    if (hipHostMalloc(p, bytes) != hipSuccess) return fail(h, PSBA_E_NOMEM, "no pinned memory (%zu bytes)", bytes);
    return PSBA_OK;
  }
  PSBA_HIP(h, hipMalloc(p, bytes));
// ... 184 lines not shown
      return fail(h, PSBA_E_INVALID, "%s: covariance of observation %d is not positive definite", __func__, a);
    const double i00 = r / det, i01 = -q / det, i11 = p / det;
    const double l00 = std::sqrt(i00), l01 = i01 / l00;
    const double t = i11 - l01 * l01;
    if (!(t > 0.0)) return fail(h, PSBA_E_INVALID, "%s: covariance of observation %d is not positive definite", __func__, a);
    w[(size_t)LENS_WSTRIDE * a] = l00;
    w[(size_t)LENS_WSTRIDE * a + 1] = l01;
    w[(size_t)LENS_WSTRIDE * a + 2] = std::sqrt(t);
  }
  if (!h->lens_w) TRY(h->lens_w.alloc(h, w.size()));
  PSBA_HIP(h, hipMemcpyAsync(h->lens_w, w.data(), sizeof(double) * w.size(), hipMemcpyHostToDevice, h->stream));
  PSBA_HIP(h, hipStreamSynchronize(h->stream));
  h->lens |= LENS_COV;
  lens_changed(h);
  return PSBA_OK;
}

int psba_lens_model(psba_handle h, int *has_distortion, int *has_covariance) {
  CHECK_H(h);
  if (has_distortion) *has_distortion = ((h->lens & LENS_DIST) || h->cnp == KD_CNP) ? 1 : 0;
  if (has_covariance) *has_covariance = (h->lens & LENS_COV) ? 1 : 0;
  return PSBA_OK;
}

static_assert(PSBA_LOSS_NONE == LOSS_NONE && PSBA_LOSS_HUBER == LOSS_HUBER && PSBA_LOSS_CAUCHY == LOSS_CAUCHY &&
                  PSBA_LOSS_SOFT_L1 == LOSS_SOFT_L1,
              "loss kinds of the C ABI and the kernels");

int psba_set_robust_loss(psba_handle h, int kind, double scale) {
  CHECK_H(h);
  TRY(lens_settable(h, __func__));
  if (kind < PSBA_LOSS_NONE || kind > PSBA_LOSS_SOFT_L1) return fail(h, PSBA_E_INVALID, "%s: unknown loss kind %d", __func__, kind);
  if (!(std::isfinite(scale) && scale > 0.0))
    return fail(h, PSBA_E_INVALID, "%s: the scale must be finite and > 0 (got %.17g)", __func__, scale);
  h->loss_kind = kind;
  h->loss_c = scale;
  if (kind == PSBA_LOSS_NONE)
    h->lens &= ~LENS_ROBUST;
  else
    h->lens |= LENS_ROBUST;
  lens_changed(h);
  return PSBA_OK;
}

int psba_robust_loss(psba_handle h, int *kind, double *scale) {
  CHECK_H(h);
  if (kind) *kind = h->loss_kind;
  if (scale) *scale = h->loss_c;
  return PSBA_OK;
}

int psba_set_fixed(psba_handle h, const unsigned char *fixed_cams, const unsigned char *fixed_pts) {
  CHECK_H(h);
  TRY(lens_settable(h, __func__));
  const int nC = h->d.nC, nP = h->d.nP;
  int nfc = 0, nfp = 0;
  for (int j = 0; fixed_cams && j < nC; j++) nfc += fixed_cams[j] ? 1 : 0;
  for (int i = 0; fixed_pts && i < nP; i++) nfp += fixed_pts[i] ? 1 : 0;
  if (h->nranks == 1 && nfc == nC && nfp == nP)
    return fail(h, PSBA_E_INVALID, "%s: every camera and every point is fixed: no free parameter is left", __func__);
  std::vector<unsigned char> fc, fp;
  DevBuf<unsigned char> new_c, new_p;
  auto stage = [&]() -> int {
    if (nfc) {
      fc.resize((size_t)nC);
      for (int j = 0; j < nC; j++) fc[j] = fixed_cams[j] ? 1 : 0;
      TRY(new_c.alloc(h, (size_t)nC));
      PSBA_HIP(h, hipMemcpyAsync(new_c, fc.data(), fc.size(), hipMemcpyHostToDevice, h->stream));
    }
    if (nfp) {
      fp.resize((size_t)nP);
      for (int i = 0; i < nP; i++) fp[i] = fixed_pts[i] ? 1 : 0;
      TRY(new_p.alloc(h, (size_t)nP));
      PSBA_HIP(h, hipMemcpyAsync(new_p, fp.data(), fp.size(), hipMemcpyHostToDevice, h->stream));
    }
    PSBA_HIP(h, hipStreamSynchronize(h->stream));
    return PSBA_OK;
  };
  const int rc = stage();
  if (rc != PSBA_OK) {
    (void)hipStreamSynchronize(h->stream);
    return rc;
  }
  h->fix_cams = std::move(new_c);
  h->fix_pts = std::move(new_p);
  h->n_fix_cams = nfc;
  h->n_fix_pts = nfp;
  h->has_fixed = nfc > 0 || nfp > 0;
  h->struct_only = nfc == nC;
  h->try_shortcut = false;
  lens_changed(h);
  return PSBA_OK;
}

int psba_fixed_counts(psba_handle h, int *n_fixed_cams, int *n_fixed_pts) {
  CHECK_H(h);
  if (n_fixed_cams) *n_fixed_cams = h->n_fix_cams;
  if (n_fixed_pts) *n_fixed_pts = h->n_fix_pts;
  return PSBA_OK;
}

int psba_set_intrinsics_mask(psba_handle h, const unsigned char *free10) {
  CHECK_H(h);
  NEED(h, h->uploaded, "no problem uploaded");
  NEED(h, h->cnp == KD_CNP, "psba_set_intrinsics_mask: PSBA_CAMERA_FREE_KD only");
  NEED(h, !h->backsub_pending, "psba_set_intrinsics_mask: a damping try is in flight (psba_backsub_wait first)");
  unsigned m = 0;
  for (int k = 0; k < 10; k++) m |= (!free10 || free10[k]) ? 1u << k : 0u;
  h->kd_mask = m;
  lens_changed(h);
  return PSBA_OK;
}

int psba_intrinsics_mask(psba_handle h, unsigned char *out10) {
  CHECK_H(h);
  NEED(h, h->uploaded, "no problem uploaded");
  NEED(h, h->cnp == KD_CNP, "psba_intrinsics_mask: PSBA_CAMERA_FREE_KD only");
  for (int k = 0; out10 && k < 10; k++) out10[k] = (h->kd_mask >> k) & 1u;
  return PSBA_OK;
}

static int groups_split(psba_ctx *h, const char *who, const std::vector<int> &rep, const double *v, int stride, int ncols,
                        int col0) {
  for (int j = 0; j < (int)rep.size(); j++)
    for (int k = 0; rep[j] != j && k < ncols; k++)
      if (memcmp(v + (size_t)stride * j + k, v + (size_t)stride * rep[j] + k, sizeof(double)) != 0)
        return fail(h, PSBA_E_INVALID, "%s: camera %d differs from camera %d, the representative of its group, in column %d "
                    "(%.17g against %.17g): members of a group hold bit-identical intrinsics",
                    who, j, rep[j], col0 + k, v[(size_t)stride * j + k], v[(size_t)stride * rep[j] + k]);
  return PSBA_OK;
}

int psba_set_intrinsics_groups(psba_handle h, const int *group_of_cam) {
  CHECK_H(h);
  NEED(h, h->uploaded, "no problem uploaded");
  NEED(h, h->cnp == KD_CNP, "psba_set_intrinsics_groups: PSBA_CAMERA_FREE_KD only");
  NEED(h, !h->backsub_pending, "psba_set_intrinsics_groups: a damping try is in flight (psba_backsub_wait first)");
  const int nC = h->d.nC;
  std::vector<int> rep((size_t)nC), order((size_t)nC);
  for (int j = 0; j < nC; j++) order[j] = j;
  if (group_of_cam)
    std::stable_sort(order.begin(), order.end(), [&](int a, int b) { return group_of_cam[a] < group_of_cam[b]; });
  int ngroups = 0;
  for (int t = 0; t < nC; t++) {
    const bool first = !group_of_cam || t == 0 || group_of_cam[order[t]] != group_of_cam[order[t - 1]];
    rep[order[t]] = first ? order[t] : rep[order[t - 1]];
    ngroups += first ? 1 : 0;
  }
  std::vector<int> gidx((size_t)nC, -1), gptr(1, 0), gmem;
  DevBuf<int> d_rep, d_gidx, d_gptr, d_gmem;
  if (ngroups < nC) {
    std::vector<double> c((size_t)h->d.nA);
    const double *src[2] = {h->cams[h->cur], h->params0};
    const char *who[2] = {"psba_set_intrinsics_groups (current parameters)", "psba_set_intrinsics_groups (the psba_reset_params copy)"};
    for (int k = 0; k < 2; k++) {
      PSBA_HIP(h, hipMemcpyAsync(c.data(), src[k], sizeof(double) * c.size(), hipMemcpyDeviceToHost, h->stream));
      PSBA_HIP(h, hipStreamSynchronize(h->stream));
      TRY(groups_split(h, who[k], rep, c.data(), KD_CNP, 10, 0));
    }
    std::vector<int> count((size_t)nC, 0);
    for (int j = 0; j < nC; j++) count[rep[j]]++;
    for (int j = 0; j < nC; j++)
      if (rep[j] == j && count[j] > 1) {
        for (int m = j; m < nC; m++)
          if (rep[m] == j) {
            gidx[m] = (int)gptr.size() - 1;
// ... 368 lines not shown
            plan.runs ? " (runs layout)" : "", h->nGroups, h->nWg, plan.real_items, plan.items.size(),
            plan.items.size() ? (double)plan.real_items / (double)plan.items.size() : 1.0,
            8e-6 * (double)plan.slab_doubles);
  return PSBA_OK;
}

static int plan_schur_blockprod(psba_ctx *h, const Upload &u) {
  int seg = KD_SEG_DEFAULT;
  if (const char *e = getenv("PSBA_FKD_SEG"))
    if (atoi(e) > 0) seg = atoi(e);
  BlockProdPlanHost plan;
  if (build_blockprod_plan(u.nC, u.nO, u.iidx, u.jidx, u.ptr.data(), seg, plan) != PSBA_OK)
    return fail(h, PSBA_E_INVALID, "%s: more than 2^31 products Y_a W_b^T", h->cnp == KD_CNP ? "PSBA_CAMERA_FREE_KD" : "PSBA_CAMERA_FREE_K");
  TRY(upload(h, h->free_blocks, plan.blocks));
  TRY(upload(h, h->free_segs, plan.segs));
  TRY(upload(h, h->free_prods, plan.prods));
  if (!plan.multi.empty()) TRY(upload(h, h->free_multi, plan.multi));
  TRY(h->free_tiles.alloc(h, (size_t)h->cnp * h->cnp * (plan.ntiles ? plan.ntiles : 1)));
  h->free_nsegs = (int)plan.segs.size();
  h->free_nmulti = (int)plan.multi.size();
  return PSBA_OK;
}

static int plan_schur(psba_ctx *h, const Upload &u) {
  if (h->solver == PSBA_SOLVER_PCG) return plan_schur_sparse(h, u);
#ifdef PSBA_BUILD_EXPERIMENTS
  TRY(plan_schur_ring(h, u));
  if (h->ring_nWg) return PSBA_OK;
#endif
  if (h->cnp != 6) return plan_schur_blockprod(h, u);
  return plan_schur_lds(h, u);
}

static int copy_inputs(psba_ctx *h, const Upload &u) {
  const Dims &d = h->d;
  std::vector<double> cc((size_t)u.nC * 9);
  for (int j = 0; j < u.nC; j++) {
    for (int k = 0; k < 5; k++) cc[(size_t)9 * j + k] = u.Kparas[5 * j + k];
    for (int k = 0; k < 4; k++) cc[(size_t)9 * j + 5 + k] = u.initrot[4 * j + k];
  }
  TRY(upload(h, h->camconst, cc));
  TRY(upload(h, h->ptr, u.ptr));
  TRY(upload(h, h->tile_pt, u.tile_pt));
  if (h->nLong) TRY(upload(h, h->long_pts, u.long_pts));
  std::vector<int4> tile_desc;
  for (int t = 0; t < d.nTilesAll; t++)
    if (u.ptr[u.tile_pt[t + 1]] - u.ptr[u.tile_pt[t]] <= TILE_OBS)
      tile_desc.push_back(make_int4(u.tile_pt[t], u.tile_pt[t + 1], u.ptr[u.tile_pt[t]], u.ptr[u.tile_pt[t + 1]]));
  if (tile_desc.empty()) tile_desc.push_back(make_int4(0, 0, 0, 0));
  TRY(upload(h, h->tile_desc, tile_desc));
  const double *cams = u.camsEx;
  std::vector<double> cam11;
  if (h->cnp != 6) {
    cam11.assign((size_t)d.nA, 0.0);
    for (int j = 0; j < u.nC; j++) {
      for (int k = 0; k < 5; k++) cam11[(size_t)h->cnp * j + k] = u.Kparas[5 * j + k];
      for (int k = 0; k < 6; k++) cam11[(size_t)h->cnp * j + h->cnp - 6 + k] = u.camsEx[6 * j + k];
    }
    cams = cam11.data();
  }
  auto H2D = [&](void *dst, const void *src, size_t bytes) {
    return hipMemcpyAsync(dst, src, bytes, hipMemcpyHostToDevice, h->stream);
  };
  PSBA_HIP(h, H2D(h->cams[0], cams, sizeof(double) * d.nA));
  PSBA_HIP(h, H2D(h->pts[0], u.pts3D, sizeof(double) * d.nB));
  PSBA_HIP(h, H2D(h->params0, cams, sizeof(double) * d.nA));
  PSBA_HIP(h, H2D(h->params0 + d.nA, u.pts3D, sizeof(double) * d.nB));
  PSBA_HIP(h, H2D(h->impts, u.impts, sizeof(double) * 2 * (size_t)d.nO));
  PSBA_HIP(h, H2D(h->iidx, u.iidx, sizeof(int) * (size_t)d.nO));
  PSBA_HIP(h, H2D(h->jidx, u.jidx, sizeof(int) * (size_t)d.nO));
  PSBA_HIP(h, hipStreamSynchronize(h->stream));
  return PSBA_OK;
}

int psba_upload_problem(psba_handle h, int nCams, int n3Dpts, int n2Dprojs, const double *Kparas,
                        const double *impts, const double *initrot, const double *camsEx,
                        const double *pts3D, const int *iidx, const int *jidx) {
  CHECK_H(h);
  Upload u{nCams, n3Dpts, n2Dprojs, Kparas, impts, initrot, camsEx, pts3D, iidx, jidx};
  TRY(build_point_csr(h, u));
  cut_tiles(u);
  PSBA_HIP(h, hipSetDevice(h->device));
  drop_problem(h);
  set_dims(h, u);
  TRY(alloc_work_buffers(h));
  if (h->cam_global || h->cnp != 6) TRY(upload_camera_index(h, u));
  TRY(plan_schur(h, u));
  TRY(copy_inputs(h, u));
  PSBA_HIP(h, hipDeviceSynchronize());
  h->uploaded = true;
  return PSBA_OK;
}

int psba_set_params(psba_handle h, const double *camsEx, const double *pts3D) {
  CHECK_H(h);
  NEED(h, h->uploaded, "no problem uploaded");
  if (!h->kd_rep_h.empty()) TRY(groups_split(h, "psba_set_params", h->kd_rep_h, camsEx, KD_CNP, 10, 0));
  PSBA_HIP(h, hipMemcpyAsync(h->cams[h->cur], camsEx, sizeof(double) * h->d.nA,
                             hipMemcpyHostToDevice, h->stream));
  PSBA_HIP(h, hipMemcpyAsync(h->pts[h->cur], pts3D, sizeof(double) * h->d.nB,
                             hipMemcpyHostToDevice, h->stream));
  PSBA_HIP(h, hipStreamSynchronize(h->stream));
  h->linearized = h->assembled = h->solved = h->backsubbed = false;
  h->ahead = h->lin_is_ahead = h->backsub_pending = h->publish_deferred = h->publish_in_k1 = false;
  h->free_obs = false;
  return PSBA_OK;
}

int psba_reset_params(psba_handle h) {
  CHECK_H(h);
  NEED(h, h->uploaded, "no problem uploaded");
  PSBA_HIP(h, hipMemcpyAsync(h->cams[h->cur], h->params0, sizeof(double) * h->d.nA, hipMemcpyDeviceToDevice,
                             h->stream));
  PSBA_HIP(h, hipMemcpyAsync(h->pts[h->cur], h->params0 + h->d.nA, sizeof(double) * h->d.nB,
                             hipMemcpyDeviceToDevice, h->stream));
  h->linearized = h->assembled = h->solved = h->backsubbed = false;
  h->ahead = h->lin_is_ahead = h->backsub_pending = h->publish_deferred = h->publish_in_k1 = false;
  h->free_obs = false;
  return PSBA_OK;
}

int psba_get_params(psba_handle h, int which, double *camsEx, double *pts3D) {
  CHECK_H(h);
  NEED(h, h->uploaded, "no problem uploaded");
  const int set = which == PSBA_PARAMS_NEW ? 1 - h->cur : h->cur;
  if (camsEx)
    PSBA_HIP(h, hipMemcpyAsync(camsEx, h->cams[set], sizeof(double) * h->d.nA,
                               hipMemcpyDeviceToHost, h->stream));
  if (pts3D)
    PSBA_HIP(h, hipMemcpyAsync(pts3D, h->pts[set], sizeof(double) * h->d.nB,
                               hipMemcpyDeviceToHost, h->stream));
  PSBA_HIP(h, hipStreamSynchronize(h->stream));
  return PSBA_OK;
}


static int fetch_scalars(psba_ctx *h) {
  PSBA_HIP(h, hipMemcpyAsync(h->h_scal, h->scal, sizeof(double) * NSCAL, hipMemcpyDeviceToHost,
                             h->stream));
  PSBA_HIP(h, hipStreamSynchronize(h->stream));
  return PSBA_OK;
}

static int enqueue_residual(psba_ctx *h, int which) {
  TRY(launch_residual(h, which, nullptr));
  if (h->comm)
    RCCL(h, ncclAllReduce(h->scal + SC_COST, h->scal + SC_COST, 1, ncclDouble, ncclSum, h->comm,
                          h->stream));
  return PSBA_OK;
}

int psba_residual(psba_handle h, int which, double *cost) {
  CHECK_H(h);
  NEED(h, h->uploaded, "no problem uploaded");
  TRY(enqueue_residual(h, which));
  TRY(fetch_scalars(h));
  if (cost) *cost = h->h_scal[SC_COST];
  return PSBA_OK;
}

int psba_linearize(psba_handle h, double coeff, double coeff_g) {
  CHECK_H(h);
  NEED(h, h->uploaded, "no problem uploaded");
  if (!(h->lin_is_ahead && coeff == h->coeff && coeff_g == h->coeff_g)) {
    h->coeff = coeff;
    h->coeff_g = coeff_g;
    TRY(launch_linearize(h, false));
    h->free_obs = h->cnp != 6;
  }
  h->lin_is_ahead = false;
  h->ahead = false;
  h->linearized = true;
  h->assembled = h->solved = h->backsubbed = false;
  return PSBA_OK;
}

static int enqueue_max_diag(psba_ctx *h) {
  if (h->comm) {
    double *tmp = h->dp;
    PSBA_HIP(h, hipMemcpyAsync(tmp, h->U, sizeof(double) * 36 * h->d.nC, hipMemcpyDeviceToDevice,
                               h->stream));
    RCCL(h, ncclAllReduce(tmp, tmp, (size_t)36 * h->d.nC, ncclDouble, ncclSum, h->comm, h->stream));
    std::swap(h->U, h->dp);
    int rc = launch_max_diag(h);
    std::swap(h->U, h->dp);
    TRY(rc);
    RCCL(h, ncclAllReduce(h->scal + SC_MAXDIAG, h->scal + SC_MAXDIAG, 1, ncclDouble, ncclMax,
                          h->comm, h->stream));
  } else {
    TRY(launch_max_diag(h));
  }
  return PSBA_OK;
}

int psba_begin(psba_handle h, double coeff, double coeff_g, double *cost, double *max_diag) {
  CHECK_H(h);
  NEED(h, h->uploaded, "no problem uploaded");
  TRY(enqueue_residual(h, PSBA_PARAMS_CUR));
  h->coeff = coeff;
  h->coeff_g = coeff_g;
  TRY(launch_linearize(h, false));
  h->free_obs = h->cnp != 6;
  h->linearized = true;
  h->assembled = h->solved = h->backsubbed = false;
  h->ahead = false;
  TRY(enqueue_max_diag(h));
  TRY(fetch_scalars(h));
  if (cost) *cost = h->h_scal[SC_COST];
  if (max_diag) *max_diag = h->h_scal[SC_MAXDIAG];
  h->lin_is_ahead = true;
  return PSBA_OK;
}

int psba_max_diag(psba_handle h, double *out) {
  CHECK_H(h);
  NEED(h, h->linearized, "psba_linearize first");
  TRY(enqueue_max_diag(h));
  TRY(fetch_scalars(h));
  if (out) *out = h->h_scal[SC_MAXDIAG];
  return PSBA_OK;
}

int psba_schur_assemble(psba_handle h, double mu) {
  CHECK_H(h);
  NEED(h, h->linearized, "psba_linearize first");
  h->mu = mu;
  h->try_shortcut = h->struct_only && h->cnp == 6 && !getenv("PSBA_FIXED_NO_SHORTCUT");
  h->cholmod_factor = false;
  if (h->try_shortcut)
    TRY(launch_struct_only_try(h, mu));
  else
    TRY(launch_schur(h, mu, false));
  h->assembled = true;
  h->solved = h->backsubbed = false;
  return PSBA_OK;
}

static int allreduce_schur(psba_ctx *h) {
  if (h->solver == PSBA_SOLVER_PCG) {
    if (h->comm)
      RCCL(h, ncclAllReduce(h->bs_val, h->bs_val, (size_t)36 * h->bs_nblk + h->d.nA, ncclDouble, ncclSum, h->comm, h->stream));
    return PSBA_OK;
  }
  if (h->packed_pending) {
    if (h->comm)
      RCCL(h, ncclAllReduce(h->redp, h->redp, h->packed_doubles, ncclDouble, ncclSum, h->comm, h->stream));
    TRY(launch_schur_expand(h));
    h->packed_pending = false;
  } else if (h->comm) {
    const size_t n = (size_t)(h->n32 + 1) * h->n32;
    RCCL(h, ncclAllReduce(h->red, h->red, n, ncclDouble, ncclSum, h->comm, h->stream));
  }
  return PSBA_OK;
}

int psba_schur_reduce(psba_handle h) {
  CHECK_H(h);
  NEED(h, h->assembled, "psba_schur_assemble first");
  if (!h->comm || h->try_shortcut) return PSBA_OK;
  ProfScope ps(h, PSBA_K_ALLREDUCE);
// ... 207 lines not shown
  h->cholmod_factor = false;
  TRY(chol_dist_finish(h));
  h->assembled = false;
  h->solved = true;
  return PSBA_OK;
}

static int ensure_trv(psba_ctx *h) {
  for (int k = 0; k < 2; k++)
    if (!h->trv[k]) TRY(h->trv[k].alloc(h, (size_t)h->d.nT));
  return PSBA_OK;
}

int psba_jmul_dots(psba_handle h, const double *x1, const double *x2, double dots[3]) {
  CHECK_H(h);
  NEED_SIX(h);
  NEED(h, h->uploaded, "no problem uploaded");
  if (!x1 || !dots) return fail(h, PSBA_E_INVALID, "psba_jmul_dots: null pointer");
  TRY(ensure_trv(h));
  const size_t bytes = sizeof(double) * (size_t)h->d.nT;
  PSBA_HIP(h, hipMemcpyAsync(h->trv[0], x1, bytes, hipMemcpyHostToDevice, h->stream));
  if (x2 && x2 != x1) PSBA_HIP(h, hipMemcpyAsync(h->trv[1], x2, bytes, hipMemcpyHostToDevice, h->stream));
  TRY(launch_jmul(h, h->trv[0], (x2 && x2 != x1) ? h->trv[1] : h->trv[0], nullptr, h->scal + SC_TR_DOTS));
  if (h->comm)
    RCCL(h, ncclAllReduce(h->scal + SC_TR_DOTS, h->scal + SC_TR_DOTS, 3, ncclDouble, ncclSum, h->comm, h->stream));
  TRY(fetch_scalars(h));
  for (int k = 0; k < 3; k++) dots[k] = h->h_scal[SC_TR_DOTS + k];
  return PSBA_OK;
}

int psba_set_solver(psba_handle h, int solver, double tol, int max_iter) {
  CHECK_H(h);
  if (solver != PSBA_SOLVER_DENSE && solver != PSBA_SOLVER_PCG) return fail(h, PSBA_E_INVALID, "unknown solver %d", solver);
  NEED(h, !h->uploaded || solver == h->solver, "psba_set_solver before psba_upload_problem (the buffers depend on it)");
  h->solver = solver;
  if (tol > 0) h->pcg_tol = tol;
  if (max_iter > 0) h->pcg_maxit = max_iter;
  return PSBA_OK;
}

int psba_pcg_info(psba_handle h, int *iters, double *relres, long long *blocks, long long *dense_blocks) {
  CHECK_H(h);
  NEED(h, h->uploaded && h->solver == PSBA_SOLVER_PCG, "PSBA_SOLVER_PCG and an uploaded problem");
  if (iters) *iters = h->pcg_iters;
  if (relres) *relres = h->pcg_relres;
  if (blocks) *blocks = h->bs_nblk;
  if (dense_blocks) *dense_blocks = (long long)h->d.nC * (h->d.nC + 1) / 2;
  return PSBA_OK;
}

int psba_get_sparse_S(psba_handle h, int *jk, double *val, double *ea) {
  CHECK_H(h);
  NEED(h, h->assembled && h->solver == PSBA_SOLVER_PCG, "psba_schur_assemble with PSBA_SOLVER_PCG first");
  NEED(h, !h->try_shortcut, "every camera is fixed: this try assembled no S (PSBA_FIXED_NO_SHORTCUT=1 keeps the general route)");
  if (jk) TRY(d2h(h, jk, h->bs_jk, sizeof(int2) * (size_t)h->bs_nblk));
  if (val) TRY(d2h(h, val, h->bs_val, sizeof(double) * 36 * (size_t)h->bs_nblk));
  if (ea) TRY(d2h(h, ea, h->bs_ea, sizeof(double) * (size_t)h->d.nA));
  return PSBA_OK;
}

int psba_set_sparse_S(psba_handle h, const double *val, const double *ea) {
  CHECK_H(h);
  NEED(h, h->assembled && h->solver == PSBA_SOLVER_PCG, "psba_schur_assemble with PSBA_SOLVER_PCG first");
  NEED(h, !h->try_shortcut, "every camera is fixed: this try assembled no S (PSBA_FIXED_NO_SHORTCUT=1 keeps the general route)");
  if (val) PSBA_HIP(h, hipMemcpyAsync(h->bs_val, val, sizeof(double) * 36 * (size_t)h->bs_nblk, hipMemcpyHostToDevice, h->stream));
  if (ea) PSBA_HIP(h, hipMemcpyAsync(h->bs_ea, ea, sizeof(double) * (size_t)h->d.nA, hipMemcpyHostToDevice, h->stream));
  PSBA_HIP(h, hipStreamSynchronize(h->stream));
  h->solved = h->backsubbed = false;
  return PSBA_OK;
}

int psba_sparse_pattern(int nCams, int n3Dpts, int n2Dprojs, const int *iidx, const int *jidx, unsigned char *flags) {
  if (nCams <= 0 || n3Dpts <= 0 || n2Dprojs <= 0 || !iidx || !jidx || !flags) return PSBA_E_INVALID;
  std::vector<int> ptr((size_t)n3Dpts + 1, 0);
  for (int a = 0; a < n2Dprojs; a++) {
    if (iidx[a] < 0 || iidx[a] >= n3Dpts || jidx[a] < 0 || jidx[a] >= nCams) return PSBA_E_INVALID;
    if (a && (iidx[a] < iidx[a - 1] || (iidx[a] == iidx[a - 1] && jidx[a] <= jidx[a - 1]))) return PSBA_E_INVALID;
    ptr[(size_t)iidx[a] + 1]++;
  }
  for (int i = 0; i < n3Dpts; i++) ptr[(size_t)i + 1] += ptr[(size_t)i];
  return psba::sparse_pattern(nCams, n2Dprojs, iidx, jidx, ptr.data(), flags);
}

int psba_set_sparse_pattern(psba_handle h, const unsigned char *flags, long long n) {
  CHECK_H(h);
  if (!flags || n <= 0) return fail(h, PSBA_E_INVALID, "psba_set_sparse_pattern: null pattern");
  NEED(h, !h->uploaded, "psba_set_sparse_pattern before psba_upload_problem (the block list depends on it)");
  h->bs_pattern.assign(flags, flags + n);
  return PSBA_OK;
}

int psba_allreduce_scalars(psba_handle h, double *v, int n) {
  CHECK_H(h);
  if (!v || n < 0 || n > 8) return fail(h, PSBA_E_INVALID, "psba_allreduce_scalars: at most 8 values");
  if (!h->comm || n == 0) return PSBA_OK;
  double *tmp = h->scal + SC_SUMS;
  PSBA_HIP(h, hipMemcpyAsync(tmp, v, sizeof(double) * (size_t)n, hipMemcpyHostToDevice, h->stream));
  RCCL(h, ncclAllReduce(tmp, tmp, (size_t)n, ncclDouble, ncclSum, h->comm, h->stream));
  return d2h(h, v, tmp, sizeof(double) * (size_t)n);
}

int psba_compute_Jmultiply(psba_handle h, const double *x, double *Jmul) {
  CHECK_H(h);
  NEED_SIX(h);
  NEED(h, h->uploaded, "no problem uploaded");
  if (!x) return fail(h, PSBA_E_INVALID, "psba_compute_Jmultiply: null pointer");
  TRY(ensure_trv(h));
  if (!h->jmul_out) TRY(h->jmul_out.alloc(h, (size_t)2 * h->d.nO));
  PSBA_HIP(h, hipMemcpyAsync(h->trv[0], x, sizeof(double) * (size_t)h->d.nT, hipMemcpyHostToDevice, h->stream));
  TRY(launch_jmul(h, h->trv[0], h->trv[0], h->jmul_out, h->scal + SC_TR_DOTS));
  return d2h(h, Jmul, h->jmul_out, sizeof(double) * 2 * (size_t)h->d.nO);
}

int psba_get_gradient(psba_handle h, double *g) {
  CHECK_H(h);
  if (h->cnp == KD_CNP) {
    NEED(h, h->linearized, "psba_linearize first");
    if (!g) return PSBA_E_INVALID;
    TRY(d2h(h, g, h->ga, sizeof(double) * (size_t)h->d.nA));
    std::vector<double> pv((size_t)9 * h->d.nP);
    TRY(d2h(h, pv.data(), h->PV, sizeof(double) * pv.size()));
    for (int i = 0; i < h->d.nP; i++)
      for (int k = 0; k < 3; k++) g[h->d.nA + 3 * (size_t)i + k] = pv[(size_t)9 * i + 6 + k];
    return PSBA_OK;
  }
  NEED_SIX(h);
  NEED(h, h->linearized, "psba_linearize first");
  if (!g) return PSBA_E_INVALID;
  TRY(ensure_trv(h));
  TRY(launch_pack_g(h, h->trv[0]));
  if (h->comm) RCCL(h, ncclAllReduce(h->trv[0], h->trv[0], (size_t)h->d.nA, ncclDouble, ncclSum, h->comm, h->stream));
  return d2h(h, g, h->trv[0], sizeof(double) * (size_t)h->d.nT);
}

int psba_get_dp(psba_handle h, double *dp) {
  CHECK_H(h);
  NEED(h, h->uploaded, "no problem uploaded");
  return d2h(h, dp, h->dp, sizeof(double) * (size_t)h->d.nT);
}

int psba_set_step(psba_handle h, const double *dp) {
  CHECK_H(h);
  NEED_SIX(h);
  NEED(h, h->uploaded, "no problem uploaded");
  if (!dp) return PSBA_E_INVALID;
  PSBA_HIP(h, hipMemcpyAsync(h->dp, dp, sizeof(double) * (size_t)h->d.nT, hipMemcpyHostToDevice, h->stream));
  TRY(launch_newp(h, h->dp));
  h->ahead = false;
  h->backsubbed = true;
  return PSBA_OK;
}

int psba_cholmod_lambda(psba_handle h, int reassemble, double *lambda, double *info3) {
  CHECK_H(h);
  NEED_SIX(h);
  NEED(h, h->uploaded, "no problem uploaded");
  if (h->nranks > 1 && !h->comm)
    return fail(h, PSBA_E_INVALID, "psba_cholmod_lambda on a rank layout needs the communicator (S must be complete)");
  NEED(h, !(h->try_shortcut && h->assembled), "a structure-only try is open (psba_schur_solve / psba_backsub first)");
  if (h->try_shortcut) {
    reassemble = 1;
    h->try_shortcut = false;
  }
  h->cholmod_factor = false;
  if (h->solver == PSBA_SOLVER_PCG) {
    NEED(h, h->linearized, "psba_linearize first");
// ... 62 lines not shown
static int d2h(psba_ctx *h, void *dst, const void *src, size_t bytes) {
  if (!dst) return PSBA_OK;
  PSBA_HIP(h, hipMemcpyAsync(dst, src, bytes, hipMemcpyDeviceToHost, h->stream));
  PSBA_HIP(h, hipStreamSynchronize(h->stream));
  return PSBA_OK;
}

static int relinearize_dump(psba_ctx *h) {
  TRY(ensure_dbg(h));
  TRY(launch_linearize(h, true));
  h->linearized = true;
  h->assembled = h->solved = h->backsubbed = false;
  return PSBA_OK;
}

static int reassemble_dump(psba_ctx *h) {
  NEED(h, h->linearized, "linearise first (compute_jacobiQT / compute_U / ...)");
  TRY(ensure_dbg(h));
  h->try_shortcut = false;
  h->cholmod_factor = false;
  TRY(launch_schur(h, h->mu_applied ? h->mu : 0.0, true));
  h->assembled = true;
  h->solved = h->backsubbed = false;
  if (h->comm) TRY(allreduce_schur(h));
  return PSBA_OK;
}

int psba_compute_exQT(psba_handle h, int which, double *ex) {
  CHECK_H(h);
  NEED(h, h->uploaded, "no problem uploaded");
  TRY(ensure_dbg(h));
  TRY(launch_residual(h, which, h->dbg_ex));
  return d2h(h, ex, h->dbg_ex, sizeof(double) * 2 * (size_t)h->d.nO);
}

int psba_compute_jacobiQT(psba_handle h, double *jac_A, double *jac_B) {
  CHECK_H(h);
  NEED(h, h->uploaded, "no problem uploaded");
  TRY(relinearize_dump(h));
  TRY(d2h(h, jac_A, h->dbg_JA, sizeof(double) * 12 * (size_t)h->d.nO));
  return d2h(h, jac_B, h->dbg_JB, sizeof(double) * 6 * (size_t)h->d.nO);
}

int psba_compute_U(psba_handle h, double coeff, double *out) {
  CHECK_H(h);
  NEED_SIX(h);
  NEED(h, h->uploaded, "no problem uploaded");
  h->coeff = coeff;
  TRY(relinearize_dump(h));
  return d2h(h, out, h->U, sizeof(double) * 36 * (size_t)h->d.nC);
}

static int download_V(psba_ctx *h, double *out, double mu) {
  if (!out) return PSBA_OK;
  std::vector<double> pv((size_t)9 * h->d.nP);
  TRY(d2h(h, pv.data(), h->PV, sizeof(double) * pv.size()));
  for (int i = 0; i < h->d.nP; i++) {
    const double *s = &pv[(size_t)9 * i];
    double *o = out + (size_t)9 * i;
    o[0] = s[0] + mu; o[1] = s[1]; o[2] = s[2];
    o[3] = s[1]; o[4] = s[3] + mu; o[5] = s[4];
    o[6] = s[2]; o[7] = s[4]; o[8] = s[5] + mu;
  }
  return PSBA_OK;
}

int psba_compute_V(psba_handle h, double coeff, double *out) {
  CHECK_H(h);
  NEED_SIX(h);
  NEED(h, h->uploaded, "no problem uploaded");
  h->coeff = coeff;
  TRY(relinearize_dump(h));
  return download_V(h, out, 0.0);
}

int psba_maxElmOfUV(psba_handle h, double *out) { return psba_max_diag(h, out); }

int psba_update_UV(psba_handle h, double mu, double *U, double *V) {
  CHECK_H(h);
  NEED_SIX(h);
  NEED(h, h->linearized, "linearise first");
  h->mu = mu;
  h->mu_applied = true;
  if (U) {
    TRY(d2h(h, U, h->U, sizeof(double) * 36 * (size_t)h->d.nC));
    for (int t = 0; t < h->d.nA; t++) U[36 * (t / 6) + 7 * (t % 6)] += mu;
  }
  return download_V(h, V, mu);
}

int psba_restore_UVdiag(psba_handle h) {
  CHECK_H(h);
  h->mu_applied = false;
  return PSBA_OK;
}

int psba_compute_Vinv(psba_handle h, double *Vinv) {
  CHECK_H(h);
  TRY(reassemble_dump(h));
  TRY(d2h(h, Vinv, h->dbg_Vinv, sizeof(double) * 9 * (size_t)h->d.nP));
  TRY(fetch_scalars(h));
  return h->h_status[0] == h->try_id ? PSBA_SINGULAR_V : PSBA_OK;
}

int psba_compute_Wblks(psba_handle h, double coeff, double *Wblks) {
  CHECK_H(h);
  NEED_SIX(h);
  NEED(h, h->uploaded, "no problem uploaded");
  h->coeff = coeff;
  TRY(relinearize_dump(h));
  return d2h(h, Wblks, h->W, sizeof(double) * 18 * (size_t)h->d.nO);
}

int psba_compute_Yblks(psba_handle h, double *Yblks) {
  CHECK_H(h);
  TRY(reassemble_dump(h));
  return d2h(h, Yblks, h->dbg_Y, sizeof(double) * 18 * (size_t)h->d.nO);
}

int psba_compute_S(psba_handle h, double *S) {
  CHECK_H(h);
  TRY(reassemble_dump(h));
  if (!S) return PSBA_OK;
  PSBA_HIP(h, hipMemcpy2DAsync(S, sizeof(double) * h->d.nA, h->red, sizeof(double) * h->n32,
                               sizeof(double) * h->d.nA, h->d.nA, hipMemcpyDeviceToHost, h->stream));
  PSBA_HIP(h, hipStreamSynchronize(h->stream));
  return PSBA_OK;
}

int psba_compute_g(psba_handle h, double coeff, double *g) {
  CHECK_H(h);
  NEED_SIX(h);
  NEED(h, h->uploaded, "no problem uploaded");
  h->coeff_g = coeff;
  TRY(relinearize_dump(h));
  if (!g) return PSBA_OK;
  TRY(d2h(h, g, h->ga, sizeof(double) * (size_t)h->d.nA));
  std::vector<double> pv((size_t)9 * h->d.nP);
  TRY(d2h(h, pv.data(), h->PV, sizeof(double) * pv.size()));
  for (int i = 0; i < h->d.nP; i++)
    for (int k = 0; k < 3; k++) g[h->d.nA + 3 * (size_t)i + k] = pv[(size_t)9 * i + 6 + k];
  return PSBA_OK;
}

int psba_compute_ea(psba_handle h, double *ea) {
  CHECK_H(h);
  TRY(reassemble_dump(h));
  return d2h(h, ea, h->red + (size_t)h->n32 * h->n32, sizeof(double) * (size_t)h->d.nA);
}

int psba_SPDinv_matVec(psba_handle h, double *dpa) {
  CHECK_H(h);
  NEED(h, h->assembled, "compute_S / compute_ea first");
  NEED(h, !h->try_shortcut, "every camera is fixed: psba_schur_assemble assembled no S (compute_S / compute_ea first)");
  h->cholmod_factor = false;
  TRY(launch_chol_solve(h));
  h->assembled = false;
  h->solved = true;
  TRY(fetch_scalars(h));
  TRY(d2h(h, dpa, h->dp, sizeof(double) * (size_t)h->d.nA));
  return h->h_status[1] == h->try_id ? PSBA_NOT_SPD : PSBA_OK;
}

static int backsub_dump(psba_ctx *h) {
  NEED(h, h->solved, "SPDinv_matVec first");
  TRY(ensure_dbg(h));
  TRY(launch_backsub(h, h->mu_applied ? h->mu : 0.0, true));
  h->backsubbed = true;
  return PSBA_OK;
}

int psba_compute_eb(psba_handle h, double *eb) {
  CHECK_H(h);
  TRY(backsub_dump(h));
  return d2h(h, eb, h->dbg_eb, sizeof(double) * 3 * (size_t)h->d.nP);
}

int psba_compute_dpb(psba_handle h, double *dp) {
  CHECK_H(h);
  TRY(backsub_dump(h));
  return d2h(h, dp, h->dp, sizeof(double) * (size_t)h->d.nT);
}

int psba_compute_newp(psba_handle h, double *new_p) {
  CHECK_H(h);
  NEED(h, h->backsubbed, "compute_dpb first");
  if (!new_p) return PSBA_OK;
  TRY(d2h(h, new_p, h->cams[1 - h->cur], sizeof(double) * (size_t)h->d.nA));
  return d2h(h, new_p + h->d.nA, h->pts[1 - h->cur], sizeof(double) * (size_t)h->d.nB);
}

int psba_update_p(psba_handle h, double *p) {
  CHECK_H(h);
  TRY(psba_accept(h));
  if (!p) return PSBA_OK;
  TRY(d2h(h, p, h->cams[h->cur], sizeof(double) * (size_t)h->d.nA));
  return d2h(h, p + h->d.nA, h->pts[h->cur], sizeof(double) * (size_t)h->d.nB);
}


int psba_partition_points(int n3Dpts, const int *iidx, int n2Dprojs, int nranks, int *pt_begin) {
  if (n3Dpts <= 0 || nranks <= 0 || !iidx || !pt_begin || n2Dprojs < 0) return PSBA_E_INVALID;
  std::vector<long long> cum((size_t)n3Dpts + 1, 0);
  for (int a = 0; a < n2Dprojs; a++) {
    if (iidx[a] < 0 || iidx[a] >= n3Dpts) return PSBA_E_INVALID;
    cum[(size_t)iidx[a] + 1]++;
  }
  for (int i = 0; i < n3Dpts; i++) cum[(size_t)i + 1] += cum[i];
  pt_begin[0] = 0;
  int p = 0;
  for (int r = 1; r < nranks; r++) {
    const long long target = (long long)n2Dprojs * r / nranks;
    while (p < n3Dpts && cum[p] < target) p++;
    int lo = pt_begin[r - 1] + 1, hi = n3Dpts - (nranks - r);
    if (n3Dpts >= nranks) {
      if (p < lo) p = lo;
      if (p > hi) p = hi;
    }
    pt_begin[r] = p;
  }
  pt_begin[nranks] = n3Dpts;
  return PSBA_OK;
}

int psba_comm_unique_id(void *id128) {
  if (!id128) return PSBA_E_INVALID;
  static_assert(sizeof(ncclUniqueId) == 128, "RCCL unique id is 128 bytes");
  ncclUniqueId id;
  if (ncclGetUniqueId(&id) != ncclSuccess) return PSBA_E_RCCL;
  memcpy(id128, &id, sizeof id);
  return PSBA_OK;
}

int psba_comm_init(psba_handle h, int nranks, int rank, const void *id128) {
  CHECK_H(h);
  if (nranks < 1 || rank < 0 || rank >= nranks || !id128)
    return fail(h, PSBA_E_INVALID, "psba_comm_init: bad rank %d / %d", rank, nranks);
  PSBA_HIP(h, hipSetDevice(h->device));
  ncclUniqueId id;
  memcpy(&id, id128, sizeof id);
  RCCL(h, ncclCommInitRank(&h->comm, nranks, id, rank));
  if (!h->stream2) {
    PSBA_HIP(h, hipStreamCreateWithFlags(&h->stream2, hipStreamNonBlocking));
    PSBA_HIP(h, hipEventCreateWithFlags(&h->k3_event, hipEventDisableTiming));
  }
  h->nranks = nranks;
  h->rank = rank;
  return PSBA_OK;
}

int psba_set_rank_layout(psba_handle h, int nranks, int rank) {
  CHECK_H(h);
  NEED(h, h->cnp == 6 || nranks <= 1, "free intrinsics (PSBA_CAMERA_FREE_K / PSBA_CAMERA_FREE_KD): single rank only");
  if (nranks < 1 || rank < 0 || rank >= nranks) return fail(h, PSBA_E_INVALID, "bad rank %d / %d", rank, nranks);
  if (h->comm) return fail(h, PSBA_E_STATE, "a communicator is attached: its layout is fixed");
  if (h->solver == PSBA_SOLVER_PCG && h->uploaded && nranks != h->nranks)
    return fail(h, PSBA_E_STATE, "PSBA_SOLVER_PCG: the rank layout is part of the block list, set it before psba_upload_problem");
  h->nranks = nranks;
  h->rank = rank;
  return PSBA_OK;
}

static bool packed_hook(psba_ctx *h) {
  return !h->comm && h->nranks > 1 && (h->nGroups > 0 || h->ring_nWg > 0) && getenv("PSBA_SCHUR_PACKED");
}

int psba_reduce_buffer_size(psba_handle h, long long *n_doubles) {
  CHECK_H(h);
  NEED(h, h->uploaded, "no problem uploaded");
  if (n_doubles) *n_doubles = packed_hook(h) ? (long long)h->packed_doubles : (long long)(h->n32 + 1) * h->n32;
  return PSBA_OK;
}

int psba_get_reduce_buffer(psba_handle h, double *out) {
  CHECK_H(h);
  NEED(h, h->assembled, "psba_schur_assemble first");
  NEED(h, !h->comm, "the reduce-buffer verbs are for handles without a communicator");
  NEED(h, h->solver != PSBA_SOLVER_PCG, "no dense reduce buffer with PSBA_SOLVER_PCG (psba_get_sparse_S)");
  NEED(h, !h->try_shortcut, "every camera is fixed: this try assembled no S (PSBA_FIXED_NO_SHORTCUT=1 keeps the general route)");
  if (packed_hook(h)) return d2h(h, out, h->redp, sizeof(double) * h->packed_doubles);
  return d2h(h, out, h->red, sizeof(double) * (size_t)(h->n32 + 1) * h->n32);
}

int psba_set_reduce_buffer(psba_handle h, const double *in) {
  CHECK_H(h);
  NEED(h, h->cnp == 6 || h->cnp == KD_CNP, SIX_ONLY);
  NEED(h, h->assembled, "psba_schur_assemble first");
  NEED(h, !h->comm, "the reduce-buffer verbs are for handles without a communicator");
  NEED(h, !h->try_shortcut, "every camera is fixed: this try assembled no S (PSBA_FIXED_NO_SHORTCUT=1 keeps the general route)");
  if (!in) return fail(h, PSBA_E_INVALID, "null buffer");
  if (packed_hook(h)) {
    PSBA_HIP(h, hipMemcpyAsync(h->redp, in, sizeof(double) * h->packed_doubles, hipMemcpyHostToDevice, h->stream));
    PSBA_HIP(h, hipStreamSynchronize(h->stream));
    h->packed_pending = true;
    h->diag_done = false;
    return PSBA_OK;
  }
  PSBA_HIP(h, hipMemcpyAsync(h->red, in, sizeof(double) * (size_t)(h->n32 + 1) * h->n32,
                             hipMemcpyHostToDevice, h->stream));
  PSBA_HIP(h, hipStreamSynchronize(h->stream));
  h->diag_done = false;
  return PSBA_OK;
}

int psba_comm_rank(psba_handle h, int *nranks, int *rank) {
  CHECK_H(h);
  if (nranks) *nranks = h->nranks;
  if (rank) *rank = h->rank;
  return PSBA_OK;
}


static int prof_flush(psba_ctx *h) {
  PSBA_HIP(h, hipStreamSynchronize(h->stream));
  for (size_t k = 0; k < h->spans_used; k++) {
    float ms = 0.f;
    if (hipEventElapsedTime(&ms, h->spans[k].a, h->spans[k].b) == hipSuccess) {
      h->prof_ms[h->spans[k].kind] += ms;
      h->prof_n[h->spans[k].kind]++;
    }
  }
  h->spans_used = 0;
  return PSBA_OK;
}

int psba_profile_enable(psba_handle h, int on) {
  CHECK_H(h);
  TRY(prof_flush(h));
  h->prof = on < 0 ? ~0u : (unsigned)on;
  while (h->prof && h->spans.size() < 512) {
    psba_ctx::Span s;
    s.kind = 0;
    if (hipEventCreateWithFlags(&s.a, hipEventDisableSystemFence) != hipSuccess ||
        hipEventCreateWithFlags(&s.b, hipEventDisableSystemFence) != hipSuccess)
      break;
    h->spans.push_back(s);
  }
  return PSBA_OK;
}

// ... 247 lines not shown
```

### psba_amd/csrc/psba_internal.h

```cpp
#pragma once
#include <hip/hip_runtime.h>
#include <rccl/rccl.h>

#include <string>
#include <vector>

#include "../../include/psba_hip.h"
#include "dev_buf.h"

namespace psba {

constexpr int TILE_OBS = 256;
constexpr int TILE_PTS = 128;
constexpr int MAX_GROUPS = 128;
constexpr int CAM_ACC = 27;
constexpr int NSCAL = 104;
constexpr int SC_NPART = 16;

enum {
  SC_COST = 0,
  SC_DP_L2 = 1,
  SC_GAIN_DEN = 2,
  SC_NEW_COST = 3,
  SC_NEWP_L2 = 4,
// ... 64 lines not shown
  int slots;
  int earow;
};
struct RingWg {
  int blk0, nblk;
  int row0, nrows;
  int copy, nsteps;
  int nwslots, pad;
  long long step0, ent0, op0, job0, lane0, bl0;
};
struct RingPlanHost {
  int nR = 0, nS = 0, nWg = 0, lat = 2;
  std::vector<int> rb;
  std::vector<RingWg> wgs;
  std::vector<RingStep> steps;
  std::vector<unsigned> entries;
  std::vector<int> ops;
  std::vector<RingJob> jobs;
  std::vector<int> lane_blk;
  std::vector<int> blk_lane0;
  long long products = 0, slots = 0, loaded_recs = 0;
};
#endif
struct SchurPlanHost {
  std::vector<unsigned long long> items;
  std::vector<SchurWg> wgs;
  std::vector<int> blockpos;
  std::vector<int> posblock;
  size_t slab_doubles = 0;
  long long real_items = 0;
  bool runs = false;
  long long tasks = 0;
  long long pair_items = 0;
};
struct BlockProdPlanHost {
  std::vector<int2> blocks;
  std::vector<int4> segs;
  std::vector<int2> prods;
  std::vector<int4> multi;
  int ntiles = 0;
  int seg_len = 0;
};
constexpr int KD_UNIT = 64;
constexpr int KD_SEG_DEFAULT = 64;
constexpr int KD_RED = 4 * 520;
constexpr int RUN_THREADS = 512;
constexpr int RUN_MAX = 32;
}

struct ProblemState {
  psba::Dims d;
  psba::DevBuf<double> camconst;
  psba::DevBuf<double> cams[2];
  psba::DevBuf<double> pts[2];
  psba::DevBuf<double> params0;
  psba::DevBuf<double> impts;
  int lens = 0;
  int loss_kind = 0;
  double loss_c = 1.0;
  psba::DevBuf<double> obs_s;
  psba::DevBuf<double> lens_kc;
  psba::DevBuf<double> lens_w;
  psba::DevBuf<unsigned char> fix_cams, fix_pts;
  int n_fix_cams = 0, n_fix_pts = 0;
  bool has_fixed = false, struct_only = false;
  bool try_shortcut = false;
  psba::DevBuf<int> iidx;
  psba::DevBuf<int> jidx;
  psba::DevBuf<int> ptr;
  psba::DevBuf<int> tile_pt;
  psba::DevBuf<int> long_pts;
  int nLong = 0;
  psba::DevBuf<int4> tile_desc;
  psba::DevBuf<double> W;
  psba::DevBuf<double> PV;
  psba::DevBuf<double> U;
  psba::DevBuf<double> ga;
  psba::DevBuf<double> W_alt, PV_alt, U_alt, ga_alt;
  bool ahead = false;
  bool lin_is_ahead = false;
  bool scal_side = false;
  psba::DevBuf<double> campart;
  int nPart = 0;
  bool cam_global = false;
  psba::DevBuf<double> camacc;
  psba::DevBuf<int> cam_obs;
  psba::DevBuf<int4> cam_units;
  int nCamUnits = 0;
  psba::DevBuf<double> red;
  int n32 = 0;
  int nGroups = 0;
  int nWg = 0;
  std::vector<int> gblk0;
  std::vector<int> gnwg;
  std::vector<int> gnblk;
  std::vector<size_t> gslab;
  psba::DevBuf<psba::ReduceGroup> gtab;
  psba::DevBuf<psba::SchurWg> wg;
  psba::DevBuf<unsigned long long> items;
  bool schur_runs = false;
  bool schur_pairs = false;
  psba::DevBuf<double> redp;
  size_t packed_doubles = 0;
  bool packed_pending = false;
  psba::DevBuf<double> diag0;
  int h_diagpos[21] = {0};
  int h_diaggrp[21] = {0};
  bool diag_done = false;
  bool cholmod_factor = false;
  psba::DevBuf<int> posblock;
  psba::DevBuf<double> slab;
  size_t packedN = 0;
  int ring_nWg = 0, ring_nS = 0;
#ifdef PSBA_BUILD_EXPERIMENTS
  psba::DevBuf<psba::RingWg> ring_wg;
  psba::DevBuf<psba::RingStep> ring_steps;
  psba::DevBuf<unsigned> ring_entries;
  psba::DevBuf<int> ring_ops;
  psba::DevBuf<psba::RingJob> ring_jobs;
  psba::DevBuf<int> ring_bl0;
  psba::DevBuf<int> ring_canon;
  psba::DevBuf<double> ring_slab;
  psba::DevBuf<double> ring_pvi;
  long long ring_products = 0, ring_slots = 0;
  size_t ring_loaded_recs = 0;
  psba::DevBuf<long long> chol_tim_ring;
#endif
  int pcg_iters = 0;
  double pcg_relres = 0.0;
  bool pcg_exhausted = false;
  long long bs_nblk = 0;
  psba::DevBuf<double> bs_val;
  double *bs_ea = nullptr;
  psba::DevBuf<int2> bs_jk;
  psba::DevBuf<int> bs_diag;
  psba::DevBuf<int> bs_rowptr;
  psba::DevBuf<int2> bs_rowent;
  psba::DevBuf<double> pcg_vec;
  psba::DevBuf<double> pcg_minv;
  psba::DevBuf<double> pcg_scal;
  psba::DevBuf<int2> own_prod;
  psba::DevBuf<psba::OwnerWave> own_waves;
  psba::DevBuf<psba::OwnerUnit> own_units;
  int own_nwaves = 0;
  long long own_products = 0;
  psba::DevBuf<int> free_cuptr;
  psba::DevBuf<double> free_Be;
  psba::DevBuf<double> free_upart;
  psba::DevBuf<double> free_Y;
  psba::DevBuf<double> free_eapart;
  psba::DevBuf<int2> free_blocks, free_prods;
  psba::DevBuf<int4> free_segs, free_multi;
  psba::DevBuf<double> free_tiles;
  int free_nsegs = 0, free_nmulti = 0;
  psba::DevBuf<double> free_red;
  unsigned kd_mask = 0x3FFu;
  std::vector<int> kd_rep_h;
  int kd_ngroups = 0;
  psba::DevBuf<int> kd_rep;
  psba::DevBuf<int> kd_gidx;
  psba::DevBuf<int> kd_gptr;
  psba::DevBuf<int> kd_gmem;
  int kd_nmg = 0;
  psba::DevBuf<double> dp;
  psba::DevBuf<double> trv[2];
  psba::DevBuf<double> jmul_out;
  psba::GraphExec chol_graph[2];
  int chol_graph_n32[2] = {0, 0};
  double *chol_graph_red[2] = {nullptr, nullptr};
  psba::DevBuf<long long> chol_tim;
  psba::DevBuf<double> chol_L;
  psba::DevBuf<double> dist_buf;
  psba::DevBuf<double> chol_ws;
  psba::DevBuf<double> dbg_ex, dbg_JA, dbg_JB, dbg_Y, dbg_Vinv, dbg_eb;

  bool uploaded = false, linearized = false, assembled = false, solved = false, backsubbed = false;
  bool backsub_pending = false;
  bool free_obs = false;
  bool publish_deferred = false, publish_in_k1 = false;
  int cur = 0;
  double coeff = 1.0, coeff_g = 1.0, mu = 0.0;
  double coeff_w = 1.0;
  bool mu_applied = false;
};

struct psba_ctx : ProblemState {
  int device = 0;
  hipStream_t stream = nullptr;
  std::string err;

  ncclComm_t comm = nullptr;
  int nranks = 1, rank = 0;

  double *h_scal_dev = nullptr;
  hipEvent_t scal_event = nullptr;
  hipStream_t stream2 = nullptr;
  hipEvent_t k3_event = nullptr;
  hipStream_t chol_side = nullptr;
  std::vector<hipEvent_t> chol_events;

  int solver = 0;
  int cnp = 6;
  double pcg_tol = 1e-10;
  int pcg_maxit = 500;
  psba::PinnedBuf<double> pcg_host;
  std::vector<unsigned char> bs_pattern;

  psba::DevBuf<double> scal;
  int *status = nullptr;
  int try_id = 0;
  double pub_seq = 0.0;
  psba::PinnedBuf<double> h_scal;
  int *h_status = nullptr;

  bool lds_attr_set = false, atomic_attr_set = false, chol_attr_set = false, lin_attr_set = false, ring_attr_set = false;

  unsigned prof = 0;
  struct Span { hipEvent_t a, b; int kind; };
  std::vector<Span> spans;
  size_t spans_used = 0;
  double prof_ms[PSBA_K_COUNT] = {0};
  int prof_n[PSBA_K_COUNT] = {0};
};

namespace psba {

int fail(psba_ctx *h, int code, const char *fmt, ...);
#define PSBA_HIP(h, call)                                                              \
  do {                                                                                 \
    hipError_t e__ = (call);                                                           \
    if (e__ != hipSuccess)                                                             \
      return psba::fail((h), PSBA_E_HIP, "%s failed: %s (%s:%d)", #call,               \
                        hipGetErrorString(e__), __FILE__, __LINE__);                   \
  } while (0)

struct ProfScope {
  psba_ctx *h;
  int idx = -1;
  ProfScope(psba_ctx *h, int kind);
  ~ProfScope();
};

int launch_linearize(psba_ctx *h, bool dump, bool ahead = false, bool publish = false);
int launch_residual(psba_ctx *h, int which, double *ex_out_dev, double *s_out_dev = nullptr);
int launch_max_diag(psba_ctx *h);
int build_schur_plan(psba_ctx *h, int nCams, int nPts, int nObs, const int *iidx, const int *jidx,
                     const int *ptr, SchurPlanHost &out);
int build_owner_plan(int nCams, int nObs, const int *iidx, const int *jidx, const int *ptr, OwnerPlanHost &out,
                     const unsigned char *pattern = nullptr);
int sparse_pattern(int nCams, int nObs, const int *iidx, const int *jidx, const int *ptr, unsigned char *flags);
#ifdef PSBA_BUILD_EXPERIMENTS
int build_ring_plan(int nCams, int nPts, int nObs, const int *iidx, const int *jidx, const int *ptr, RingPlanHost &out,
                    bool force = false);
int launch_schur_ring(psba_ctx *h, double mu, bool dump);
struct SchurLdsArgs;
bool launch_schur_lds_mode(int mode, dim3 G, dim3 B, size_t lds, hipStream_t s, const SchurLdsArgs &a);
#endif
int launch_schur(psba_ctx *h, double mu, bool dump);
int launch_schur_expand(psba_ctx *h);
int launch_chol_solve(psba_ctx *h);
int mirror_refused(psba_ctx *h);
int build_blockprod_plan(int nCams, int nObs, const int *iidx, const int *jidx, const int *ptr, int seg_len,
                         BlockProdPlanHost &out);
int launch_linearize_free(psba_ctx *h, bool ahead, bool publish);
int launch_residual_free(psba_ctx *h, int which);
int launch_max_diag_free(psba_ctx *h);
int launch_schur_free(psba_ctx *h, double mu);
int launch_backsub_free(psba_ctx *h, double mu);
int launch_bsr_finalize(psba_ctx *h, double mu);
int launch_pcg_solve(psba_ctx *h);
int launch_bsr_gershgorin(psba_ctx *h, double *lambda, double *info3);
int launch_chol_graph(psba_ctx *h);
int chol_dist_shape(psba_ctx *h, int *NB, int *blocked);
int chol_shape(psba_ctx *h, int *out8);
int chol_dist_exchange_plan(int n32, int NB, int nranks, int JE, long long (*out)[4], int cap);
int chol_dist_begin(psba_ctx *h);
int chol_dist_superpanel(psba_ctx *h, int J);
int chol_dist_block(psba_ctx *h, int B, double *buf_dev, int set);
int chol_dist_finish(psba_ctx *h);
int launch_backsub(psba_ctx *h, double mu, bool dump);
int launch_publish_scal(psba_ctx *h, hipStream_t s);
int launch_struct_only_try(psba_ctx *h, double mu);
int launch_jmul(psba_ctx *h, const double *x1_dev, const double *x2_dev, double *out1_dev, double *dots_dev);
int launch_pack_g(psba_ctx *h, double *g_dev);
int launch_newp(psba_ctx *h, double *dp_dev);
int launch_cholmod(psba_ctx *h, double *out4_dev);

}
```

### psba_amd/csrc/schur_lds_args.h

```cpp
#pragma once
#include "psba_internal.h"

namespace psba {

constexpr int SCHUR_THREADS = 1024;
constexpr int BLK_STRIDE = 37;

struct SchurLdsArgs {
  const double *W, *PV;
  const SchurWg *wg;
  const unsigned long long *items;
  double *slab;
  int *status;
  double *dbg_Y, *dbg_Vinv;
  double mu;
  int nWg, try_id;
  double *diag0;
  int diag_grp[21], diag_pos[21];
};

}
```

Baseline: 2103 M-obs/s.

## Fold deferred camera-sum reduction into the Schur LDS kernel prologue

When linearization runs ahead on the single-rank dense path, the per-workgroup camera partial sums are no longer reduced by a separate k_cam_reduce launch. The pending reduction is recorded and executed inside the Schur kernel prologue, with workgroups folding camera chunks into U and ga before zeroing their LDS. Other consumers of U and ga settle the owed sums first. This removes a kernel launch and a serial dependency, but adds bookkeeping for owed state and extra prologue work and LDS in the Schur kernel.

```diff
diff --git a/include/psba_hip.h b/include/psba_hip.h
--- a/include/psba_hip.h
+++ b/include/psba_hip.h
@@ -223,6 +223,10 @@
 int psba_sparse_pattern(int nCams, int n3Dpts, int n2Dprojs, const int *iidx, const int *jidx, unsigned char *flags);
 int psba_set_sparse_pattern(psba_handle h, const unsigned char *flags, long long n);
 
+int psba_cam_fold_chunk(int nCams, int chunk, int *out3);
+int psba_cam_sums_owed(psba_handle h, int *owed);
+int psba_cam_sums_reference(psba_handle h, double *U, double *ga);
+
 int psba_chol_dist_shape(psba_handle h, int *n32, int *NB, int *sharded);
 int psba_chol_shape(psba_handle h, int *out8);
 int psba_chol_dist_exchange_plan(int n32, int NB, int nranks, int JE, long long *out4, int cap);
diff --git a/psba_amd/capi.py b/psba_amd/capi.py
--- a/psba_amd/capi.py
+++ b/psba_amd/capi.py
@@ -147,6 +147,9 @@
     ("psba_set_sparse_S", C.c_int, [_h, _dp, _dp]),
     ("psba_sparse_pattern", C.c_int, [C.c_int, C.c_int, C.c_int, _ip, _ip, C.POINTER(C.c_ubyte)]),
     ("psba_set_sparse_pattern", C.c_int, [_h, C.POINTER(C.c_ubyte), C.c_longlong]),
+    ("psba_cam_fold_chunk", C.c_int, [C.c_int, C.c_int, _ip]),
+    ("psba_cam_sums_owed", C.c_int, [_h, _ip]),
+    ("psba_cam_sums_reference", C.c_int, [_h, _dp, _dp]),
     ("psba_set_camera_model", C.c_int, [_h, C.c_int]),
     ("psba_camera_block", C.c_int, [_h, _ip]),
     ("psba_set_distortion", C.c_int, [_h, _dp]),
@@ -291,6 +294,14 @@
         raise PsbaError(rc, f"psba_convert_bal_kd({bal_file}) failed")
 
 
+def cam_fold_chunk(n_cams, chunk):
+    out = np.zeros(3, dtype=np.int32)
+    rc = lib.psba_cam_fold_chunk(int(n_cams), int(chunk), _i(out))
+    if rc != 0:
+        raise PsbaError(rc, "psba_cam_fold_chunk failed")
+    return int(out[0]), int(out[1]), int(out[2])
+
+
 def partition_points(n_pts, iidx, nranks):
     iidx = _c(iidx, np.int32)
     out = np.zeros(nranks + 1, dtype=np.int32)
@@ -603,6 +614,16 @@
     def accept(self):
         self._ck(lib.psba_accept(self._h))
 
+    def cam_sums_reference(self):
+        U, ga = np.empty(36 * self.nC), np.empty(6 * self.nC)
+        self._ck(lib.psba_cam_sums_reference(self._h, _d(U), _d(ga)))
+        return U, ga
+
+    def cam_sums_owed(self):
+        v = C.c_int()
+        self._ck(lib.psba_cam_sums_owed(self._h, C.byref(v)))
+        return v.value
+
     def _out(self, fn, n, *pre):
         out = np.empty(n)
         rc = self._ck(fn(self._h, *pre, _d(out)))
diff --git a/psba_amd/csrc/kernels_backsub.hip b/psba_amd/csrc/kernels_backsub.hip
--- a/psba_amd/csrc/kernels_backsub.hip
+++ b/psba_amd/csrc/kernels_backsub.hip
@@ -355,6 +355,10 @@
 
 int launch_backsub(psba_ctx *h, double mu, bool dump) {
   if (h->cnp != 6) return dump ? mirror_refused(h) : launch_backsub_free(h, mu);
+  {
+    const int rc = settle_cam_sums(h);
+    if (rc != PSBA_OK) return rc;
+  }
   const Dims &d = h->d;
   BackArgs a;
   a.W = h->W;
diff --git a/psba_amd/csrc/kernels_linearize.hip b/psba_amd/csrc/kernels_linearize.hip
--- a/psba_amd/csrc/kernels_linearize.hip
+++ b/psba_amd/csrc/kernels_linearize.hip
@@ -582,7 +582,7 @@
 }
 
 template <int LM>
-static void enqueue_linearize(psba_ctx *h, const LinArgs &a, const RobustLoss &rl, const FixedMask &fm, bool dump, bool v1, size_t lds, double *Uo, double *gao) {
+static void enqueue_linearize(psba_ctx *h, const LinArgs &a, const RobustLoss &rl, const FixedMask &fm, bool dump, bool v1, size_t lds, double *Uo, double *gao, bool defer) {
   const Dims &d = h->d;
   if (h->cam_global) {
     const int grid = d.nTiles < 2048 ? d.nTiles : 2048;
@@ -622,9 +622,32 @@
         hipLaunchKernelGGL((k_linearize_long<false, false, LM>), dim3(h->nLong), dim3(TILE_OBS), 0, h->stream, a, h->long_pts, slab, rl, fm);
       nslab++;
     }
-    hipLaunchKernelGGL(k_cam_reduce, dim3(d.nC), dim3(1024), 0, h->stream, h->campart, nslab, d.nC, h->coeff,
-                       h->coeff_g, Uo, gao);
-  }
+    h->cam_last = {Uo, gao, nslab, h->coeff, h->coeff_g};
+    if (defer)
+      h->cam_owed = {Uo, gao, nslab, h->coeff, h->coeff_g};
+    else
+      hipLaunchKernelGGL(k_cam_reduce, dim3(d.nC), dim3(1024), 0, h->stream, h->campart, nslab, d.nC, h->coeff,
+                         h->coeff_g, Uo, gao);
+  }
+}
+
+int launch_cam_reduce_into(psba_ctx *h, double *U_dev, double *ga_dev) {
+  const ProblemState::CamSumRecord &r = h->cam_last;
+  hipLaunchKernelGGL(k_cam_reduce, dim3(h->d.nC), dim3(1024), 0, h->stream, h->campart, r.nslab, h->d.nC, r.coeff, r.coeff_g,
+                     U_dev, ga_dev);
+  PSBA_HIP(h, hipGetLastError());
+  return PSBA_OK;
+}
+
+int settle_cam_sums(psba_ctx *h, bool alt_too) {
+  if (!h->cam_owed.U || (!alt_too && h->cam_owed.U != h->U.get())) return PSBA_OK;
+  const ProblemState::CamSumRecord r = h->cam_owed;
+  h->cam_owed = {};
+  ProfScope ps(h, PSBA_K_LINEARIZE);
+  hipLaunchKernelGGL(k_cam_reduce, dim3(h->d.nC), dim3(1024), 0, h->stream, h->campart, r.nslab, h->d.nC, r.coeff,
+                     r.coeff_g, r.U, r.ga);
+  PSBA_HIP(h, hipGetLastError());
+  return PSBA_OK;
 }
 
 int launch_linearize(psba_ctx *h, bool dump, bool ahead, bool publish) {
@@ -673,6 +696,13 @@
     h->lin_attr_set = true;
   }
   double *Uo = ahead ? h->U_alt : h->U, *gao = ahead ? h->ga_alt : h->ga;
+  if (h->cam_owed.U == h->U.get() && Uo != h->U.get()) {
+    const int rc = settle_cam_sums(h);
+    if (rc != PSBA_OK) return rc;
+  }
+  h->cam_owed = {};
+  const bool defer = ahead && h->cam_fold && !h->cam_global && !dump && !h->has_fixed && h->nranks == 1 && !h->comm &&
+               h->solver == PSBA_SOLVER_DENSE && h->nGroups > 0 && h->ring_nWg == 0 && !getenv("PSBA_SCHUR_ATOMIC");
   {
     ProfScope ps(h, PSBA_K_LINEARIZE);
     if (h->cam_global)
@@ -680,7 +710,7 @@
     else if (h->nLong)
       PSBA_HIP(h, hipMemsetAsync(h->campart + (size_t)h->nPart * d.nC * CAM_ACC, 0, sizeof(double) * CAM_ACC * (size_t)d.nC,
                                  h->stream));
-    lens_dispatch_fixed(h->lens, h->has_fixed, [&](auto m) { enqueue_linearize<decltype(m)::value>(h, a, rl, fm, dump, v1, lds, Uo, gao); });
+    lens_dispatch_fixed(h->lens, h->has_fixed, [&](auto m) { enqueue_linearize<decltype(m)::value>(h, a, rl, fm, dump, v1, lds, Uo, gao, defer); });
     if (h->has_fixed)
       hipLaunchKernelGGL(k_fixed_diag, dim3((d.nC + d.nP + 255) / 256), dim3(256), 0, h->stream, fm, d.nC, d.nP, h->coeff,
                          h->rank == 0 ? h->coeff : 0.0, Uo, gao, a.PV);
@@ -711,6 +741,10 @@
 
 int launch_max_diag(psba_ctx *h) {
   if (h->cnp != 6) return launch_max_diag_free(h);
+  {
+    const int rc = settle_cam_sums(h);
+    if (rc != PSBA_OK) return rc;
+  }
   PSBA_HIP(h, hipMemsetAsync(h->scal + SC_MAXDIAG, 0, sizeof(double), h->stream));
   int grid = (h->d.nP + 255) / 256;
   if (grid > 512) grid = 512;
diff --git a/psba_amd/csrc/kernels_schur.hip b/psba_amd/csrc/kernels_schur.hip
--- a/psba_amd/csrc/kernels_schur.hip
+++ b/psba_amd/csrc/kernels_schur.hip
@@ -205,6 +205,66 @@
   }
 }
 
+constexpr int FOLD_TEAM = 256, FOLD_SEQ = 32, FOLD_ENT = 7, FOLD_LOADS = 24;
+
+template <int NT>
+__device__ __forceinline__ void schur_prologue(const SchurLdsArgs &p, double *sPart, int nzero) {
+  const int tid = threadIdx.x;
+  const int nchunks = p.campart ? 4 * p.nC : 0;
+  if ((int)blockIdx.x >= nchunks) {
+    for (int t = tid; t < nzero; t += NT) sPart[t] = 0.0;
+    __syncthreads();
+    return;
+  }
+  const int team = tid / FOLD_TEAM, tt = tid % FOLD_TEAM, s = tt / FOLD_ENT, el = tt % FOLD_ENT;
+  const int nteams = p.nWg * (NT / FOLD_TEAM);
+  const size_t stride = (size_t)p.nC * CAM_ACC;
+  for (int c0 = blockIdx.x; c0 < nchunks; c0 += nteams) {
+    const int c = c0 + team * p.nWg;
+    const CamChunk ch = c < nchunks ? cam_fold_chunk(c, p.nC) : CamChunk{0, 0, 0};
+    const bool active = s < FOLD_SEQ && el < ch.ne;
+    const unsigned off = (unsigned)s * (unsigned)stride + (unsigned)(ch.cam * CAM_ACC + ch.e0 + el);
+    double x[FOLD_LOADS];
+#pragma unroll
+    for (int k = 0; k < FOLD_LOADS; k++)
+      x[k] = active && s + FOLD_SEQ * k < p.nslab ? (p.campart + (size_t)(FOLD_SEQ * k) * stride)[off] : 0.0;
+    if (c0 == (int)blockIdx.x) {
+      for (int t = NT + tid; t < nzero; t += NT) sPart[t] = 0.0;
+    } else {
+      __syncthreads();
+    }
+    double acc = 0.0;
+#pragma unroll
+    for (int k = 0; k < FOLD_LOADS; k++)
+      if (s + FOLD_SEQ * k < p.nslab) acc += x[k];
+    if (active)
+      for (int q = s + FOLD_SEQ * FOLD_LOADS; q < p.nslab; q += FOLD_SEQ) acc += (p.campart + (size_t)(q - s) * stride)[off];
+    sPart[tid] = acc;
+    __syncthreads();
+    if (tt < ch.ne) {
+      double *col = sPart + team * FOLD_TEAM + tt;
+      double t = col[0];
+      for (int q = 1; q < FOLD_SEQ; q++) t += col[FOLD_ENT * q];
+      for (int q = 0; q < FOLD_SEQ; q++) col[FOLD_ENT * q] = 0.0;
+      const int e = ch.e0 + tt;
+      if (e < 21) {
+        int lo = 0, k = e;
+        while (k >= 6 - lo) {
+          k -= 6 - lo;
+          lo++;
+        }
+        const int hi = lo + k;
+        const double u = p.coeff * t;
+        p.U[36 * (size_t)ch.cam + 6 * lo + hi] = u;
+        p.U[36 * (size_t)ch.cam + 6 * hi + lo] = u;
+      } else {
+        p.ga[6 * (size_t)ch.cam + e - 21] = p.coeff_g * t;
+      }
+    }
+  }
+  __syncthreads();
+}
+
 template <bool DUMP>
 __global__ __launch_bounds__(SCHUR_THREADS) void k_schur_lds(SchurLdsArgs p) {
   extern __shared__ double sPart[];
@@ -212,8 +272,7 @@
   int w = blockIdx.x;
   if ((p.nWg & 7) == 0) w = (blockIdx.x & 7) * (p.nWg >> 3) + (blockIdx.x >> 3);
   const SchurWg wg = p.wg[w];
-  for (int t = tid; t < BLK_STRIDE * wg.nblk; t += SCHUR_THREADS) sPart[t] = 0.0;
-  __syncthreads();
+  schur_prologue<SCHUR_THREADS>(p, sPart, BLK_STRIDE * wg.nblk);
 
 #ifdef PSBA_BUILD_EXPERIMENTS
   {
@@ -317,8 +376,7 @@
   int w = blockIdx.x;
   if ((p.nWg & 7) == 0) w = (blockIdx.x & 7) * (p.nWg >> 3) + (blockIdx.x >> 3);
   const SchurWg wg = p.wg[w];
-  for (int t = tid; t < BLK_STRIDE * wg.nblk; t += RUN_THREADS) sPart[t] = 0.0;
-  __syncthreads();
+  schur_prologue<RUN_THREADS>(p, sPart, BLK_STRIDE * wg.nblk);
   double acc[36];
 #pragma unroll
   for (int k = 0; k < 36; k++) acc[k] = 0.0;
@@ -685,6 +743,31 @@
   for (int b = 0; b < 21; b++) {
     a.diag_grp[b] = h->h_diaggrp[b];
     a.diag_pos[b] = h->h_diagpos[b];
+  }
+  const char *mode_env = getenv("PSBA_SCHUR_MODE");
+  const int mode = mode_env ? atoi(mode_env) : 0;
+  bool modes_kernel = false;
+#ifdef PSBA_BUILD_EXPERIMENTS
+  modes_kernel = !h->schur_runs && !dump && mode > 0 && !h->schur_pairs;
+#endif
+  a.campart = nullptr;
+  a.U = a.ga = nullptr;
+  a.coeff = a.coeff_g = 0.0;
+  a.nslab = 0;
+  a.nC = d.nC;
+  if (h->cam_owed.U == h->U.get()) {
+    if (dump || modes_kernel) {
+      const int rc = settle_cam_sums(h);
+      if (rc != PSBA_OK) return rc;
+    } else {
+      a.campart = h->campart;
+      a.U = h->cam_owed.U;
+      a.ga = h->cam_owed.ga;
+      a.coeff = h->cam_owed.coeff;
+      a.coeff_g = h->cam_owed.coeff_g;
+      a.nslab = h->cam_owed.nslab;
+      h->cam_owed = {};
+    }
   }
   SchurReduceArgs r;
   r.slab = h->slab;
@@ -714,7 +797,8 @@
     npos += h->gnblk[g];
     if (h->gnblk[g] > worst) worst = h->gnblk[g];
   }
-  const size_t lds = sizeof(double) * BLK_STRIDE * (size_t)worst;
+  size_t lds = sizeof(double) * BLK_STRIDE * (size_t)worst;
+  if (a.campart && lds < sizeof(double) * SCHUR_THREADS) lds = sizeof(double) * SCHUR_THREADS;
   int most = 1;
   for (int g = 0; g < h->nGroups; g++) most = h->gnwg[g] > most ? h->gnwg[g] : most;
   r.grp16 = h->gtab;
@@ -728,8 +812,6 @@
     ProfScope pp(h, pair ? PSBA_K_SCHUR : -1);
     {
       ProfScope ps(h, pair ? -1 : PSBA_K_SCHUR);
-      const char *m = getenv("PSBA_SCHUR_MODE");
-      const int mode = m ? atoi(m) : 0;
       const dim3 G(h->nWg), B(SCHUR_THREADS);
       bool launched = false;
       if (h->schur_runs) {
@@ -741,9 +823,10 @@
         launched = true;
       }
 #ifdef PSBA_BUILD_EXPERIMENTS
-      if (!launched && !dump && mode > 0 && !h->schur_pairs) launched = launch_schur_lds_mode(mode, G, B, lds, h->stream, a);
+      if (!launched && modes_kernel) launched = launch_schur_lds_mode(mode, G, B, lds, h->stream, a);
 #endif
       (void)mode;
+      (void)modes_kernel;
       if (launched) {
       } else if (dump)
         hipLaunchKernelGGL((k_schur_lds<true>), G, B, lds, h->stream, a);
@@ -800,6 +883,11 @@
   h->try_id++;
   h->diag_done = false;
   h->packed_pending = false;
+  const bool lds_route = h->solver != PSBA_SOLVER_PCG && h->ring_nWg == 0 && h->nGroups > 0 && !getenv("PSBA_SCHUR_ATOMIC");
+  if (!lds_route) {
+    const int rc = settle_cam_sums(h);
+    if (rc != PSBA_OK) return rc;
+  }
   if (h->solver == PSBA_SOLVER_PCG) {
     if (dump) return fail(h, PSBA_E_INVALID, "the sba_func.h mirror verbs need the dense S: PSBA_SOLVER_DENSE");
     return launch_schur_sparse(h, mu);
diff --git a/psba_amd/csrc/kernels_tr.hip b/psba_amd/csrc/kernels_tr.hip
--- a/psba_amd/csrc/kernels_tr.hip
+++ b/psba_amd/csrc/kernels_tr.hip
@@ -529,6 +529,10 @@
 
 int launch_pack_g(psba_ctx *h, double *g_dev) {
   const size_t n = (size_t)h->d.nT;
+  {
+    const int rc = settle_cam_sums(h);
+    if (rc != PSBA_OK) return rc;
+  }
   hipLaunchKernelGGL(k_pack_g, dim3((unsigned)((n + 255) / 256)), dim3(256), 0, h->stream, h->ga, h->PV, h->d.nA, h->d.nP,
                      g_dev);
   PSBA_HIP(h, hipGetLastError());
diff --git a/psba_amd/csrc/psba_api.cpp b/psba_amd/csrc/psba_api.cpp
--- a/psba_amd/csrc/psba_api.cpp
+++ b/psba_amd/csrc/psba_api.cpp
@@ -10,6 +10,7 @@
 
 #include "camera_model.h"
 #include "psba_internal.h"
+#include "schur_lds_args.h"
 
 using namespace psba;
 
@@ -360,6 +361,7 @@
     (void)hipStreamSynchronize(h->stream);
     return rc;
   }
+  TRY(settle_cam_sums(h, true));
   h->fix_cams = std::move(new_c);
   h->fix_pts = std::move(new_p);
   h->n_fix_cams = nfc;
@@ -894,6 +896,7 @@
   cut_tiles(u);
   PSBA_HIP(h, hipSetDevice(h->device));
   drop_problem(h);
+  if (const char *e = getenv("PSBA_CAM_FOLD")) h->cam_fold = atoi(e) != 0;
   set_dims(h, u);
   TRY(alloc_work_buffers(h));
   if (h->cam_global || h->cnp != 6) TRY(upload_camera_index(h, u));
@@ -988,6 +991,7 @@
 }
 
 static int enqueue_max_diag(psba_ctx *h) {
+  TRY(settle_cam_sums(h));
   if (h->comm) {
     double *tmp = h->dp;
     PSBA_HIP(h, hipMemcpyAsync(tmp, h->U, sizeof(double) * 36 * h->d.nC, hipMemcpyDeviceToDevice,
@@ -1361,6 +1365,32 @@
   return psba::sparse_pattern(nCams, n2Dprojs, iidx, jidx, ptr.data(), flags);
 }
 
+int psba_cam_fold_chunk(int nCams, int chunk, int *out3) {
+  if (nCams <= 0 || chunk < 0 || chunk >= 4 * nCams || !out3) return PSBA_E_INVALID;
+  const CamChunk c = cam_fold_chunk(chunk, nCams);
+  out3[0] = c.cam;
+  out3[1] = c.e0;
+  out3[2] = c.ne;
+  return PSBA_OK;
+}
+
+int psba_cam_sums_owed(psba_handle h, int *owed) {
+  CHECK_H(h);
+  if (owed) *owed = !h->cam_owed.U ? 0 : h->cam_owed.U == h->U.get() ? 1 : 2;
+  return PSBA_OK;
+}
+
+int psba_cam_sums_reference(psba_handle h, double *U, double *ga) {
+  CHECK_H(h);
+  NEED_SIX(h);
+  NEED(h, h->cam_last.U, "no linearization with per-workgroup camera slabs has run");
+  DevBuf<double> tmp;
+  TRY(tmp.alloc(h, (size_t)42 * h->d.nC));
+  TRY(launch_cam_reduce_into(h, tmp, tmp + (size_t)36 * h->d.nC));
+  TRY(d2h(h, U, tmp, sizeof(double) * 36 * (size_t)h->d.nC));
+  return d2h(h, ga, tmp + (size_t)36 * h->d.nC, sizeof(double) * (size_t)h->d.nA);
+}
+
 int psba_set_sparse_pattern(psba_handle h, const unsigned char *flags, long long n) {
   CHECK_H(h);
   if (!flags || n <= 0) return fail(h, PSBA_E_INVALID, "psba_set_sparse_pattern: null pattern");
@@ -1589,6 +1619,7 @@
   NEED(h, h->linearized, "linearise first");
   h->mu = mu;
   h->mu_applied = true;
+  TRY(settle_cam_sums(h));
   if (U) {
     TRY(d2h(h, U, h->U, sizeof(double) * 36 * (size_t)h->d.nC));
     for (int t = 0; t < h->d.nA; t++) U[36 * (t / 6) + 7 * (t % 6)] += mu;
@@ -1746,6 +1777,7 @@
   PSBA_HIP(h, hipSetDevice(h->device));
   ncclUniqueId id;
   memcpy(&id, id128, sizeof id);
+  TRY(settle_cam_sums(h, true));
   RCCL(h, ncclCommInitRank(&h->comm, nranks, id, rank));
   if (!h->stream2) {
     PSBA_HIP(h, hipStreamCreateWithFlags(&h->stream2, hipStreamNonBlocking));
@@ -1763,6 +1795,7 @@
   if (h->comm) return fail(h, PSBA_E_STATE, "a communicator is attached: its layout is fixed");
   if (h->solver == PSBA_SOLVER_PCG && h->uploaded && nranks != h->nranks)
     return fail(h, PSBA_E_STATE, "PSBA_SOLVER_PCG: the rank layout is part of the block list, set it before psba_upload_problem");
+  TRY(settle_cam_sums(h, true));
   h->nranks = nranks;
   h->rank = rank;
   return PSBA_OK;
diff --git a/psba_amd/csrc/psba_internal.h b/psba_amd/csrc/psba_internal.h
--- a/psba_amd/csrc/psba_internal.h
+++ b/psba_amd/csrc/psba_internal.h
@@ -170,6 +170,13 @@
   bool scal_side = false;
   psba::DevBuf<double> campart;
   int nPart = 0;
+  struct CamSumRecord {
+    double *U = nullptr, *ga = nullptr;
+    int nslab = 0;
+    double coeff = 1.0, coeff_g = 1.0;
+  } cam_owed;
+  CamSumRecord cam_last;
+  bool cam_fold = true;
   bool cam_global = false;
   psba::DevBuf<double> camacc;
   psba::DevBuf<int> cam_obs;
@@ -332,6 +339,8 @@
 int launch_linearize(psba_ctx *h, bool dump, bool ahead = false, bool publish = false);
 int launch_residual(psba_ctx *h, int which, double *ex_out_dev, double *s_out_dev = nullptr);
 int launch_max_diag(psba_ctx *h);
+int launch_cam_reduce_into(psba_ctx *h, double *U_dev, double *ga_dev);
+int settle_cam_sums(psba_ctx *h, bool alt_too = false);
 int build_schur_plan(psba_ctx *h, int nCams, int nPts, int nObs, const int *iidx, const int *jidx,
                      const int *ptr, SchurPlanHost &out);
 int build_owner_plan(int nCams, int nObs, const int *iidx, const int *jidx, const int *ptr, OwnerPlanHost &out,
diff --git a/psba_amd/csrc/schur_lds_args.h b/psba_amd/csrc/schur_lds_args.h
--- a/psba_amd/csrc/schur_lds_args.h
+++ b/psba_amd/csrc/schur_lds_args.h
@@ -17,6 +17,27 @@
   int nWg, try_id;
   double *diag0;
   int diag_grp[21], diag_pos[21];
+  const double *campart;
+  double *U, *ga;
+  double coeff, coeff_g;
+  int nslab, nC;
 };
 
+struct CamChunk {
+  int cam, e0, ne;
+};
+__host__ __device__ inline CamChunk cam_fold_chunk(int c, int nC) {
+  const int g = c >> 5, full = nC >> 3;
+  int j, q;
+  if (g < full) {
+    q = (c & 31) >> 3;
+    j = 8 * g + (c & 7);
+  } else {
+    const int r = nC & 7, cc = c - 32 * full;
+    q = cc / r;
+    j = 8 * full + cc % r;
+  }
+  return CamChunk{j, 7 * q, q < 3 ? 7 : 6};
 }
+
+}
```

Result: faster. 2140 M-obs/s (median of 6 runs) (+1.8%).
